# endiqq/Multi-Feature-ViT

Hardware: AMD Instinct MI355X
Metric: images/sec (two-stream 224^2 vit_small MF-CA train step) (higher is better)
Workload: dtype bf16x3 (split bf16 hi+lo operands, 3 MFMAs per product, f32 accumulate)

## Files before the change

### include/mfvit.h

```cpp
#ifndef MFVIT_H
#define MFVIT_H
#include <stddef.h>
#include <stdint.h>

#ifdef __cplusplus
extern "C" {
#endif

typedef void* mfvit_stream_t;

#define MFVIT_OK 0
#define MFVIT_EINVAL (-22)
#define MFVIT_ENOSYS (-38)
#define MFVIT_ELAUNCH (-5)

#define MFVIT_F32 0
#define MFVIT_BF16 1
#define MFVIT_BF16X3 2
#define MFVIT_F16 3
#define MFVIT_X3F16 4

int mfvit_abi_version(void);
const char* mfvit_build_info(void);

typedef struct mfvit_vit_cfg {
    int dtype;
    int batch;
    int img_h, img_w;
    int dim;
    int depth;
    int heads;
    int mlp_dim;
    int save_for_backward;
    int stop_grad_conv1;
    float ln_eps;
    int token_input;
    int tokens;
    int use_pos;
    int act;
    float p_embd, p_attn, p_resid;
    uint32_t seed_lo, seed_hi;
    int stream_share;
} mfvit_vit_cfg;

size_t mfvit_vit_param_count(const mfvit_vit_cfg* cfg);
int mfvit_vit_param_layout(const mfvit_vit_cfg* cfg, int64_t out[9]);

size_t mfvit_vit_shadow_bytes(const mfvit_vit_cfg* cfg);
int mfvit_vit_prepare_shadow(const mfvit_vit_cfg* cfg, const float* params, void* shadow, mfvit_stream_t stream);

size_t mfvit_vit_workspace_bytes(const mfvit_vit_cfg* cfg);

int mfvit_vit_forward(const mfvit_vit_cfg* cfg, const float* params, const void* shadow, const float* img, void* workspace,
                      float* features, mfvit_stream_t stream);

int mfvit_vit_backward(const mfvit_vit_cfg* cfg, const float* params, const void* shadow, void* workspace, const float* dfeatures,
                       float* dparams, int stage_hi, int stage_lo, mfvit_stream_t stream);

typedef struct mfvit_vit_drop {
    float drop;
    float attn_drop;
    const float* drop_path;
    uint64_t seed;
} mfvit_vit_drop;
size_t mfvit_vit_workspace_bytes_drop(const mfvit_vit_cfg* cfg, const mfvit_vit_drop* drop);
int mfvit_vit_forward_drop(const mfvit_vit_cfg* cfg, const mfvit_vit_drop* drop, const float* params, const void* shadow, const float* img,
                           void* workspace, float* features, mfvit_stream_t stream);
int mfvit_vit_backward_drop(const mfvit_vit_cfg* cfg, const mfvit_vit_drop* drop, const float* params, const void* shadow, void* workspace,
                            const float* dfeatures, float* dparams, int stage_hi, int stage_lo, mfvit_stream_t stream);

size_t mfvit_vit_workspace_bytes_ex(const mfvit_vit_cfg* cfg, const mfvit_vit_drop* drop, int want_dimg);
int mfvit_vit_backward_ex(const mfvit_vit_cfg* cfg, const mfvit_vit_drop* drop, const float* params, const void* shadow, void* workspace,
                          const float* dfeatures, float* dparams, float* dimg, int stage_hi, int stage_lo, mfvit_stream_t stream);

typedef struct mfvit_vit_attn_req {
    uint64_t blocks;
    int fuse;
    int cls_only;
    float* maps;
    float* rollout;
    void* scratch;
} mfvit_vit_attn_req;
size_t mfvit_vit_attn_scratch_bytes(const mfvit_vit_cfg* cfg, const mfvit_vit_attn_req* req);
int mfvit_vit_forward_attn(const mfvit_vit_cfg* cfg, const mfvit_vit_attn_req* req, const float* params, const void* shadow,
                           const float* img, void* workspace, float* features, mfvit_stream_t stream);

typedef struct mfvit_vit_rel_req {
    uint64_t blocks;
    float* maps;
    float* relevance;
    void* scratch;
} mfvit_vit_rel_req;
size_t mfvit_vit_rel_scratch_bytes(const mfvit_vit_cfg* cfg, const mfvit_vit_rel_req* req);
int mfvit_vit_backward_rel(const mfvit_vit_cfg* cfg, const mfvit_vit_rel_req* req, const float* params, const void* shadow, void* workspace,
                           const float* dfeatures, mfvit_stream_t stream);

int mfvit_gpt_forward(const mfvit_vit_cfg* cfg, const float* params, const void* shadow, const float* tokens, void* workspace, float* out,
                      mfvit_stream_t stream);
int mfvit_gpt_backward(const mfvit_vit_cfg* cfg, const float* params, const void* shadow, void* workspace, const float* dout, float* dparams,
                       float* dtokens, mfvit_stream_t stream);

int mfvit_linear_fwd(int dtype, int epilogue, const void* x, int64_t ldx, const void* w, int64_t ldw, const float* bias, void* y,
                     int64_t ldy, void* y2, int64_t ldy2, int M, int N, int K, mfvit_stream_t stream);
int mfvit_linear_dgrad_act(int dtype, const void* dy, int64_t lddy, const void* wt, int64_t ldwt, const void* act_grad, int64_t ldg,
                           void* dx, int64_t lddx, int M, int N, int K, mfvit_stream_t stream);
int mfvit_linear_wgrad(int dtype, const void* dy, int64_t lddy, const void* x, int64_t ldx, float* dw, int64_t lddw, int M, int N, int K,
                       mfvit_stream_t stream);
#define MFVIT_WGRAD_SCRATCH_FLOATS (384 * 128 * 128)
int mfvit_linear_wgrad_ws(int dtype, const void* dy, int64_t lddy, const void* x, int64_t ldx, float* dw, int64_t lddw, int M, int N,
                          int K, float* scratch, mfvit_stream_t stream);
int mfvit_linear_wgrad_pair(int dtype, const void* dy_a, int64_t lddy_a, const void* x_a, int64_t ldx_a, float* dw_a, int64_t lddw_a, float* dbias_a,
                            int Na, const void* dy_b, int64_t lddy_b, const void* x_b, int64_t ldx_b, float* dw_b, int64_t lddw_b, int Nb, int M, int K,
                            mfvit_stream_t stream);
int mfvit_linear_res_ln_fwd(int dtype, const void* a, int64_t lda, const void* w, int64_t ldw, const float* bias, const float* res,
                            int64_t ldres, float* x_out, void* y, int y_f32, const float* gamma, const float* beta, float eps,
                            float* mean, float* rstd, int M, int K, mfvit_stream_t stream);
int mfvit_linear_dgrad_ln_bwd(int dtype, const void* dy, int64_t lddy, const void* wt, int64_t ldwt, const float* x, const float* mean,
                              const float* rstd, const float* gamma, const float* dres, float* dx, void* dx_t, float* dgamma,
                              float* dbeta, float* dcol, int M, int K, mfvit_stream_t stream);
#define MFVIT_ROWP_SCRATCH_FLOATS (264 * 7 * 12 * 512)
int mfvit_linear_res_ln_fwd_ws(int dtype, const void* a, int64_t lda, const void* w, int64_t ldw, const float* bias, const float* res,
                               int64_t ldres, float* x_out, void* y, int y_f32, const float* gamma, const float* beta, float eps,
                               float* mean, float* rstd, int M, int K, float* scratch, mfvit_stream_t stream);
int mfvit_linear_dgrad_ln_bwd_ws(int dtype, const void* dy, int64_t lddy, const void* wt, int64_t ldwt, const float* x, const float* mean,
                                 const float* rstd, const float* gamma, const float* dres, float* dx, void* dx_t, float* dgamma,
                                 float* dbeta, float* dcol, int M, int K, float* scratch, mfvit_stream_t stream);
int mfvit_attention_qkv_dtype(int dtype, int T, int head_dim);
int mfvit_attention_fwd(int dtype, const void* qkv, void* out, float* lse, int B, int T, int H, int head_dim, mfvit_stream_t stream);
int mfvit_attention_bwd(int dtype, const void* qkv, const void* out, const void* dout, const float* lse, void* dqkv, float* dbias_qkv,
                        int B, int T, int H, int head_dim, mfvit_stream_t stream);
int mfvit_attention_drop_fwd(int dtype, const void* qkv, void* out, float* lse, int B, int T, int H, int head_dim, float p, uint64_t seed,
                             uint32_t site, mfvit_stream_t stream);
int mfvit_attention_drop_bwd(int dtype, const void* qkv, const void* out, const void* dout, const float* lse, void* dqkv, int B, int T, int H,
                             int head_dim, float p, uint64_t seed, uint32_t site, mfvit_stream_t stream);
int mfvit_dropout_mask(float p, uint64_t seed, uint32_t site, int64_t n, uint8_t* keep, mfvit_stream_t stream);
int mfvit_layernorm_fwd(int dtype, const float* x, void* y, int y_f32, const float* gamma, const float* beta, float eps, float* mean,
                        float* rstd, int rows, int N, mfvit_stream_t stream);
int mfvit_layernorm_bwd(int dtype, const float* dy, const float* x, const float* mean, const float* rstd, const float* gamma,
                        const float* dres, float* dx, void* dx_t, float* dgamma, float* dbeta, float* dcol, int rows, int N,
                        mfvit_stream_t stream);
int mfvit_cast_transpose(int dtype, const float* src, void* dst, void* dst_t, int R, int C, mfvit_stream_t stream);
int mfvit_head_fwd(const float* x, int64_t ldx, const float* w, const float* b, float* y, int64_t ldy, int M, int N, int K, int accumulate,
                   mfvit_stream_t stream);
int mfvit_head_bwd(const float* dy, int64_t lddy, const float* x, int64_t ldx, const float* w, float* dx, int64_t lddx, int dx_accumulate,
                   float* dw, float* db, int M, int N, int K, mfvit_stream_t stream);
int mfvit_cross_entropy(const float* logits, const int64_t* target, float* loss_mean, float* dlogits, int64_t* preds, int B, int C,
                        mfvit_stream_t stream);
int mfvit_cross_entropy_soft(const float* logits, const int64_t* target, const int32_t* partner, const float* lam, float smoothing,
                             float* loss_mean, float* dlogits, int64_t* preds, int B, int C, mfvit_stream_t stream);

int mfvit_batch_mix(const float* a, const float* b, float* out_a, float* out_b, const int32_t* desc, const float* lam, int n, int C, int H,
                    int W, mfvit_stream_t stream);

int mfvit_input_transform(const uint8_t* src, const int64_t* desc, const int32_t* tables, int n, int S, int crop, const float* mean3,
                          const float* std3, float* out, mfvit_stream_t stream);
int mfvit_input_transform_rect(const uint8_t* src, const int64_t* desc, const int32_t* tables, int n, int S, int out_h, int out_w,
                               const float* mean3, const float* std3, float* out, mfvit_stream_t stream);

size_t mfvit_input_photometric_workspace_bytes(int n, int S);
int mfvit_input_photometric(const uint8_t* src, const int64_t* desc, const int32_t* tables, const int32_t* photo, int n, int S, int max_radius,
                            void* workspace, const float* mean3, const float* std3, float* out, mfvit_stream_t stream);

int mfvit_eval_counts(const float* scores, int64_t ld, const int64_t* labels, int n, int C, uint64_t* confusion, int64_t* preds,
                      uint64_t* u2, uint64_t* npos, mfvit_stream_t stream);

typedef struct mfvit_fusion_cfg {
    int batch;
    int tokens;
    int dim;
    int heads;
    int num_classes;
    float eps_pre;
    float eps_post;
} mfvit_fusion_cfg;

size_t mfvit_fusion_param_count(const mfvit_fusion_cfg* cfg);
size_t mfvit_fusion_workspace_bytes(const mfvit_fusion_cfg* cfg);
int mfvit_fusion_forward(const mfvit_fusion_cfg* cfg, const float* params, const float* f_cxr, const float* f_enh, const float* hw_cxr,
                         const float* hb_cxr, const float* hw_enh, const float* hb_enh, void* workspace, float* fused, float* x_cxr,
                         float* x_enh, mfvit_stream_t stream);
int mfvit_fusion_backward(const mfvit_fusion_cfg* cfg, const float* params, const float* f_cxr, const float* f_enh, const float* hw_cxr,
                          const float* hw_enh, void* workspace, const float* dfused, const float* dx_cxr, const float* dx_enh,
                          float* dparams, float* df_cxr, float* df_enh, float* dhw_cxr, float* dhb_cxr, float* dhw_enh, float* dhb_enh,
                          mfvit_stream_t stream);

size_t mfvit_fusion_ex_param_count(const mfvit_fusion_cfg* cfg, int cross_attn_depth, int pool_mean);
size_t mfvit_fusion_ex_workspace_bytes(const mfvit_fusion_cfg* cfg, int cross_attn_depth, int pool_mean);
int mfvit_fusion_ex_forward(const mfvit_fusion_cfg* cfg, int cross_attn_depth, int pool_mean, const float* params, const float* f_cxr,
                            const float* f_enh, const float* hw_cxr, const float* hb_cxr, const float* hw_enh, const float* hb_enh,
                            void* workspace, float* fused, float* x_cxr, float* x_enh, mfvit_stream_t stream);
int mfvit_fusion_ex_backward(const mfvit_fusion_cfg* cfg, int cross_attn_depth, int pool_mean, const float* params, const float* f_cxr,
                             const float* f_enh, const float* hw_cxr, const float* hw_enh, void* workspace, const float* dfused,
                             const float* dx_cxr, const float* dx_enh, float* dparams, float* df_cxr, float* df_enh, float* dhw_cxr,
                             float* dhb_cxr, float* dhw_enh, float* dhb_enh, mfvit_stream_t stream);

int mfvit_prenorm_xattn_forward(const mfvit_fusion_cfg* cfg, const float* params, const float* x_own, const float* x_oth,
                                void* workspace, float* out, mfvit_stream_t stream);
int mfvit_prenorm_xattn_backward(const mfvit_fusion_cfg* cfg, const float* params, const float* x_own, const float* x_oth,
                                 void* workspace, const float* dout, float* dparams, float* dx_own, float* dx_oth,
                                 mfvit_stream_t stream);

int mfvit_xattn_forward(const mfvit_fusion_cfg* cfg, const float* params, const float* x, void* workspace, float* out,
                        mfvit_stream_t stream);
int mfvit_xattn_backward(const mfvit_fusion_cfg* cfg, const float* params, const float* x, void* workspace, const float* dout,
                         float* dparams, float* dx, mfvit_stream_t stream);

int mfvit_prof_enable(int class_mask);
int mfvit_set_wgrad_stream(int enabled);
int mfvit_set_stream_share(int n);
int mfvit_prof_collect(double* out, int ncls);
int mfvit_prof_collect_tags(double* out, int ntags);
const char* mfvit_prof_class_name(int cls);

int mfvit_bn_stats(int dtype, const void* x, int n, int C, float* mean, float* m2, mfvit_stream_t stream);
int mfvit_bn_combine(const float* means, const float* m2s, const float* counts, int W, int C, float eps, float momentum, float* mean,
                     float* invstd, float* running_mean, float* running_var, mfvit_stream_t stream);
int mfvit_bn_apply(int dtype, const void* x, const float* mean, const float* invstd, const float* gamma, const float* beta, int relu,
                   void* y, int n, int C, mfvit_stream_t stream);
int mfvit_bn_bwd_sums(int dtype, const void* dy, const void* x, const void* y, const float* mean, const float* invstd, int relu, int n,
                      int C, float* s1, float* s2, mfvit_stream_t stream);
int mfvit_bn_bwd_apply(int dtype, const void* dy, const void* x, const void* y, const float* mean, const float* invstd, const float* gamma,
                       int relu, const float* S1, const float* S2, float inv_count, void* dx, int n, int C, mfvit_stream_t stream);
int mfvit_l2norm_fwd(const float* x, float* y, float* inv_norm, int n, int C, float eps, mfvit_stream_t stream);
int mfvit_l2norm_bwd(const float* dy, const float* y, const float* inv_norm, float* dx, int n, int C, mfvit_stream_t stream);
int mfvit_rowdot(const float* a, const float* b, float* out, int64_t ldo, float scale, int n, int C, mfvit_stream_t stream);
int mfvit_cross_entropy_rows(const float* logits, int64_t ld, const int64_t* target, float* loss_mean, float* lse, float* dlogits,
// ... 21 lines not shown
```

### multi-feature-vit_amd/csrc/elementwise.hip

```cpp
#include "kernels.h"

namespace mfvit {

template <typename T>
__global__ void im2col16_kernel(const float* __restrict__ img, T* __restrict__ P, int B, int Hh, int Ww) {
    const int gh = Hh / 16, gw = Ww / 16;
    const long total = (long)B * gh * gw * 3 * 16 * 2;
    for (long q = blockIdx.x * (long)blockDim.x + threadIdx.x; q < total; q += (long)gridDim.x * blockDim.x) {
        const int half = q & 1;
        long r = q >> 1;
        const int py = r % 16; r /= 16;
        const int c = r % 3; r /= 3;
        const int pw = r % gw; r /= gw;
        const int ph = r % gh; r /= gh;
        const int b = (int)r;
        const float* s = img + (((long)b * 3 + c) * Hh + ph * 16 + py) * Ww + pw * 16 + half * 8;
        const float4 v0 = *(const float4*)s, v1 = *(const float4*)(s + 4);
        const int k = c * 256 + py * 16 + half * 8;
        T* d = P + ((long)(b * gh + ph) * gw + pw) * 768 * elems_per<T>::value + (is_split<T>::value ? split_col(k) : k);
        if constexpr (sizeof(T) == 2) {
            typedef typename Vec4<T>::elem E;
            const float f[8] = {v0.x, v0.y, v0.z, v0.w, v1.x, v1.y, v1.z, v1.w};
            typename Vec8<T>::type o, l;
#pragma unroll
// ... 395 lines not shown
#pragma unroll
    for (int k = 0; k < 4; ++k) {
        const int q = threadIdx.x + 256 * k, r = q >> 4, c = (q & 15) * 4;
        float4 v = make_float4(0.f, 0.f, 0.f, 0.f);
        if (r0 + r < R && c0 + c < C) {
            v = *(const float4*)(src + (long)(r0 + r) * C + c0 + c);
            if (dst) store_elem4<T>(dst + (long)(r0 + r) * C * elems_per<T>::value, c0 + c, v.x, v.y, v.z, v.w);
        }
        tile[r][c] = v.x;
        tile[r][c + 1] = v.y;
        tile[r][c + 2] = v.z;
        tile[r][c + 3] = v.w;
    }
    __syncthreads();
    if (dstT) {
#pragma unroll
        for (int k = 0; k < 4; ++k) {
            const int q = threadIdx.x + 256 * k, c = q >> 4, r = (q & 15) * 4;
            if (r0 + r < R && c0 + c < C)
                store_elem4<T>(dstT + (long)(c0 + c) * R * elems_per<T>::value, r0 + r, tile[r][c], tile[r + 1][c], tile[r + 2][c], tile[r + 3][c]);
        }
    }
}
int cast_transpose_batched(int dtype, const float* src, void* dst, void* dstT, int R, int C, int nb, long s_src, long s_dst, long s_dstT,
                           hipStream_t st) {
    const dim3 grid((C + 63) / 64, (R + 63) / 64, nb);
    if (R % 4 == 0 && C % 4 == 0 && s_src % 4 == 0 && s_dst % 16 == 0 && s_dstT % 16 == 0 &&
        (((uintptr_t)src | (uintptr_t)dst | (uintptr_t)dstT) & 15) == 0 && !(dtype == MFVIT_BF16X3 && ((dst && C % 32) || (dstT && R % 32)))) {
        switch (dtype) {
            case MFVIT_BF16: MFVIT_LAUNCH(cast_transpose4_kernel<bf16>, grid, dim3(256), 0, st, src, (bf16*)dst, (bf16*)dstT, R, C, s_src, s_dst, s_dstT); break;
            case MFVIT_BF16X3: MFVIT_LAUNCH(cast_transpose4_kernel<sbf16>, grid, dim3(256), 0, st, src, (sbf16*)dst, (sbf16*)dstT, R, C, s_src, s_dst, s_dstT); break;
            case MFVIT_F16: MFVIT_LAUNCH(cast_transpose4_kernel<f16>, grid, dim3(256), 0, st, src, (f16*)dst, (f16*)dstT, R, C, s_src, s_dst, s_dstT); break;
            case MFVIT_F32: MFVIT_LAUNCH(cast_transpose4_kernel<float>, grid, dim3(256), 0, st, src, (float*)dst, (float*)dstT, R, C, s_src, s_dst, s_dstT); break;
            default: return MFVIT_EINVAL;
        }
        MFVIT_CHECK_LAUNCH();
        return MFVIT_OK;
    }
    if (dtype == MFVIT_BF16)
        MFVIT_LAUNCH(cast_transpose_kernel<bf16>, grid, dim3(256), 0, st, src, (bf16*)dst, (bf16*)dstT, R, C, s_src, s_dst, s_dstT);
    else if (dtype == MFVIT_BF16X3) {
        if ((dst && C % 32) || (dstT && R % 32)) return MFVIT_EINVAL;
        MFVIT_LAUNCH(cast_transpose_kernel<sbf16>, grid, dim3(256), 0, st, src, (sbf16*)dst, (sbf16*)dstT, R, C, s_src, s_dst, s_dstT);
    } else if (dtype == MFVIT_F16)
        MFVIT_LAUNCH(cast_transpose_kernel<f16>, grid, dim3(256), 0, st, src, (f16*)dst, (f16*)dstT, R, C, s_src, s_dst, s_dstT);
    else if (dtype == MFVIT_F32)
        MFVIT_LAUNCH(cast_transpose_kernel<float>, grid, dim3(256), 0, st, src, (float*)dst, (float*)dstT, R, C, s_src, s_dst, s_dstT);
    else
        return MFVIT_EINVAL;
    MFVIT_CHECK_LAUNCH();
    return MFVIT_OK;
}
int cast_transpose(int dtype, const float* src, void* dst, void* dstT, int R, int C, hipStream_t st) {
    return cast_transpose_batched(dtype, src, dst, dstT, R, C, 1, 0, 0, 0, st);
}

__global__ __launch_bounds__(256) void linear_small_fwd_kernel(const float* __restrict__ x, long ldx, const float* __restrict__ W,
                                                               const float* __restrict__ b, float* __restrict__ y, long ldy, int M, int N,
                                                               int K, int accumulate) {
    const int o = blockIdx.x * 4 + (threadIdx.x >> 6), lane = threadIdx.x & 63;
    if (o >= M * N) return;
    const int m = o / N, n = o % N;
    float s = 0.f;
    for (int k = lane; k < K; k += 64) s = fmaf(x[(long)m * ldx + k], W[(long)n * K + k], s);
    s = wave_sum(s);
    if (lane == 0) {
        s += b ? b[n] : 0.f;
        if (accumulate) y[(long)m * ldy + n] += s; else y[(long)m * ldy + n] = s;
    }
}
__global__ __launch_bounds__(256) void linear_small_bwd_kernel(const float* __restrict__ dy, long lddy, const float* __restrict__ x, long ldx,
                                                               const float* __restrict__ W, float* __restrict__ dx, long lddx,
                                                               int dx_accumulate, float* __restrict__ dW, float* __restrict__ db, int M,
                                                               int N, int K) {
    const long id = blockIdx.x * (long)blockDim.x + threadIdx.x;
    if (dx && id < (long)M * K) {
        const int m = id / K, k = id % K;
        float s = 0.f;
        for (int n = 0; n < N; ++n) s = fmaf(dy[(long)m * lddy + n], W[(long)n * K + k], s);
        if (dx_accumulate) dx[(long)m * lddx + k] += s; else dx[(long)m * lddx + k] = s;
    }
    if (dW && id < (long)N * K) {
        const int n = id / K, k = id % K;
        float s = 0.f;
        for (int m = 0; m < M; ++m) s = fmaf(dy[(long)m * lddy + n], x[(long)m * ldx + k], s);
        dW[(long)n * K + k] += s;
    }
    if (db && id < N) {
        float s = 0.f;
        for (int m = 0; m < M; ++m) s += dy[(long)m * lddy + id];
        db[id] += s;
    }
}
int linear_small_fwd(const float* x, long ldx, const float* W, const float* b, float* y, long ldy, int M, int N, int K, int accumulate,
                     hipStream_t st) {
    MFVIT_LAUNCH(linear_small_fwd_kernel, dim3((M * N + 3) / 4), dim3(256), 0, st, x, ldx, W, b, y, ldy, M, N, K, accumulate);
    MFVIT_CHECK_LAUNCH();
    return MFVIT_OK;
}
int linear_small_bwd(const float* dy, long lddy, const float* x, long ldx, const float* W, float* dx, long lddx, int dx_accumulate, float* dW,
                     float* db, int M, int N, int K, hipStream_t st) {
    long work = (long)M * K;
    if ((long)N * K > work) work = (long)N * K;
    MFVIT_LAUNCH(linear_small_bwd_kernel, dim3((unsigned)((work + 255) / 256)), dim3(256), 0, st, dy, lddy, x, ldx, W, dx, lddx,
                       dx_accumulate, dW, db, M, N, K);
    MFVIT_CHECK_LAUNCH();
    return MFVIT_OK;
}

__global__ __launch_bounds__(1024) void ce_small_kernel(const float* __restrict__ logits, const long* __restrict__ target, float* __restrict__ loss_mean,
                                                        float* __restrict__ dlogits, long* __restrict__ preds, int B, int C) {
    __shared__ float red[16];
    float li = 0.f;
    for (int b = threadIdx.x; b < B; b += 1024) {
        const float* z = logits + (long)b * C;
        float m = z[0];
        int am = 0;
        for (int c = 1; c < C; ++c) if (z[c] > m) { m = z[c]; am = c; }
        float s = 0.f;
        for (int c = 0; c < C; ++c) s += __expf(z[c] - m);
        const float lse = m + __logf(s);
        const int t = (int)target[b];
        li += (lse - z[t]) / (float)B;
        if (dlogits)
            for (int c = 0; c < C; ++c) dlogits[(long)b * C + c] = (__expf(z[c] - lse) - (c == t ? 1.f : 0.f)) / (float)B;
        if (preds) preds[b] = am;
    }
    li = wave_sum(li);
    if ((threadIdx.x & 63) == 0) red[threadIdx.x >> 6] = li;
    __syncthreads();
    if (threadIdx.x == 0) {
        float t = 0.f;
#pragma unroll
        for (int i = 0; i < 16; ++i) t += red[i];
        *loss_mean = t;
    }
}
int ce_small(const float* logits, const long* target, float* loss_mean, float* dlogits, long* preds, int B, int C, hipStream_t st) {
    if (C > 64 || C < 1) return MFVIT_EINVAL;
    MFVIT_LAUNCH(ce_small_kernel, dim3(1), dim3(1024), 0, st, logits, target, loss_mean, dlogits, preds, B, C);
    MFVIT_CHECK_LAUNCH();
    return MFVIT_OK;
}

__global__ void add_rows_kernel(float* __restrict__ dst, long ldd, const float* __restrict__ src, long lds_, int rows, int N) {
    const long id = blockIdx.x * (long)blockDim.x + threadIdx.x;
    if (id < (long)rows * N) dst[(id / N) * ldd + id % N] += src[(id / N) * lds_ + id % N];
}
int add_rows(float* dst, long ldd, const float* src, long lds_, int rows, int N, hipStream_t st) {
    MFVIT_LAUNCH(add_rows_kernel, dim3((unsigned)(((long)rows * N + 255) / 256)), dim3(256), 0, st, dst, ldd, src, lds_, rows, N);
    MFVIT_CHECK_LAUNCH();
    return MFVIT_OK;
}
__global__ void axpy_kernel(float* __restrict__ y, const float* __restrict__ x, float a, long n) {
    const long i = blockIdx.x * (long)blockDim.x + threadIdx.x;
    if (i < n) y[i] = fmaf(a, x[i], y[i]);
}
int axpy(float* y, const float* x, float a, long n, hipStream_t st) {
    MFVIT_LAUNCH(axpy_kernel, dim3((unsigned)((n + 255) / 256)), dim3(256), 0, st, y, x, a, n);
    MFVIT_CHECK_LAUNCH();
    return MFVIT_OK;
}
__global__ __launch_bounds__(1024) void colsum_rows_kernel(const float* __restrict__ x, long ld, float* __restrict__ out, int rows,
                                                           int row_stride, int row_off, int N) {
    const int n = blockIdx.x * 64 + (threadIdx.x & 63), sub = threadIdx.x >> 6;
    __shared__ float sm[16][64];
    float s = 0.f;
    if (n < N) {
#pragma unroll 4
        for (int r = sub; r < rows; r += 16) s += x[((long)r * row_stride + row_off) * ld + n];
    }
    sm[sub][threadIdx.x & 63] = s;
    __syncthreads();
    if (sub == 0 && n < N) {
        s = 0.f;
#pragma unroll
        for (int i = 0; i < 16; ++i) s += sm[i][threadIdx.x];
        out[n] += s;
    }
}
int colsum_rows(const float* x, long ld, float* out, int rows, int row_stride, int row_off, int N, hipStream_t st) {
    MFVIT_LAUNCH(colsum_rows_kernel, dim3((N + 63) / 64), dim3(1024), 0, st, x, ld, out, rows, row_stride, row_off, N);
    MFVIT_CHECK_LAUNCH();
    return MFVIT_OK;
}

__global__ __launch_bounds__(256) void batch_sum_kernel(const float* __restrict__ x, float* __restrict__ out, int B, long n) {
    const long i = blockIdx.x * 256L + threadIdx.x;
    if (i >= n) return;
    float s = 0.f;
    for (int b = 0; b < B; ++b) s += x[(long)b * n + i];
    out[i] += s;
}
int batch_sum(const float* x, float* out, int B, long n, hipStream_t st) {
    MFVIT_LAUNCH(batch_sum_kernel, dim3((unsigned)((n + 255) / 256)), dim3(256), 0, st, x, out, B, n);
    MFVIT_CHECK_LAUNCH();
    return MFVIT_OK;
}

__global__ __launch_bounds__(256) void dropout_mask_kernel(DropP drop, long n, unsigned char* __restrict__ out) {
    const long i = (long)blockIdx.x * 256 + threadIdx.x;
    if (i < n) out[i] = drop_mul(drop, (unsigned)i) != 0.f;
}
int dropout_mask(DropP drop, long n, unsigned char* out, hipStream_t st) {
    if (n <= 0 || n >= (1L << 32)) return MFVIT_EINVAL;
    MFVIT_LAUNCH(dropout_mask_kernel, dim3((unsigned)((n + 255) / 256)), dim3(256), 0, st, drop, n, out);
    MFVIT_CHECK_LAUNCH();
    return MFVIT_OK;
}

}
```

### multi-feature-vit_amd/csrc/gemm.hip

```cpp
#include "kernels.h"
#include "prof.h"

#include <stdlib.h>

#include <type_traits>

namespace mfvit {




template <typename T, int EPI, int DEEP = 0>
__global__ __launch_bounds__(256, 2) void gemm_nt_tile_kernel(GemmP p) {
    constexpr int BM = 128, BN = 128, BKB = 128, WM = 2, WN = 2, NTHR = WM * WN * 64;
    typedef NtLoop<T, BM, BN, BKB, WM, WN> Loop;
    extern __shared__ __attribute__((aligned(16))) char lds[];
    apply_batch<T>(p, sizeof(T));
    const int ntn = p.N / BN;
    const int ntm = (p.M + BM - 1) / BM;
    const int bid = xcd_remap(blockIdx.x, ntn * ntm);
    const int m0 = (bid / ntn) * BM, n0 = (bid % ntn) * BN;
    f32x16 acc[Loop::TM][Loop::TN];
    if constexpr (DEEP == 12) {
        NtLoopDeep<T, BM, BN, BKB, WM, WN, 2, true>::run(p, m0, n0, lds, acc);
// ... 739 lines not shown
    typedef STile<T, BN, KR> TA;
    typedef STile<T, BK2, KR> TB;
    constexpr int STAGE = TA::BYTES + TB::BYTES;
    extern __shared__ __attribute__((aligned(16))) char lds[];
    apply_batch<T>(p, 4);
    const int tid = threadIdx.x, lane = tid & 63, wave = tid >> 6;
    const int wm = wave >> 1, wn = wave & 1;
    constexpr bool SPLIT = is_split<T>::value;
    constexpr int EP = elems_per<T>::value;
    const int ntk = p.K * EP / BK2;
    int tile = blockIdx.x, split = blockIdx.y;
    if (gridDim.y == 1 && p.splits > 1) {
        const int tiles = ntk * (p.N * EP / BN);
        const int lin = xcd_remap(blockIdx.x, gridDim.x);
        split = lin / tiles;
        tile = lin % tiles;
    }
    const int n0 = (tile / ntk) * BN, k0 = (tile % ntk) * BK2;
    int chunk = (p.M + p.splits - 1) / p.splits;
    chunk = (chunk + KR - 1) / KR * KR;
    const int mbeg = split * chunk;
    const int mend = min(p.M, mbeg + chunk);
    if (mbeg >= mend) return;
    const T* A = (const T*)p.A;
    const T* X = (const T*)p.W;
    SStage<T, BN, KR, NT> sa;
    SStage<T, BK2, KR, NT> sb;
    f32x16 acc[2][2];
#pragma unroll
    for (int i = 0; i < 2; ++i)
#pragma unroll
        for (int j = 0; j < 2; ++j)
#pragma unroll
            for (int r = 0; r < 16; ++r) acc[i][j][r] = 0.f;
    const bool do_cs = p.cs0 != nullptr && k0 == 0 && wn == 0;
    f32x16 bacc[2];
    typename MmaTraits<T>::frag_t ones;
    if constexpr (sizeof(T) == 2) {
        typedef typename Vec4<T>::elem E16;
#pragma unroll
        for (int j = 0; j < 8; ++j) ones[j] = (E16)1.0f;
    } else {
        ones = 1.0f;
    }
#pragma unroll
    for (int i = 0; i < 2; ++i)
#pragma unroll
        for (int r = 0; r < 16; ++r) bacc[i][r] = 0.f;
    const int nst = (mend - mbeg + KR - 1) / KR;
    const int nfull = (mend - mbeg) / KR;
    auto load_stage = [&](int stg) {
        if (stg < nfull) {
            sa.template load<REMAP, false>(A, p.lda, mbeg + stg * KR, mend, n0, tid, p.orow_in, p.orow_out, p.orow_off);
            sb.template load<false, false>(X, p.ldw, mbeg + stg * KR, mend, k0, tid);
        } else {
            sa.template load<REMAP, true>(A, p.lda, mbeg + stg * KR, mend, n0, tid, p.orow_in, p.orow_out, p.orow_off);
            sb.template load<false, true>(X, p.ldw, mbeg + stg * KR, mend, k0, tid);
        }
    };
    auto main_loop = [&](auto cs_tag) {
        constexpr bool CS = decltype(cs_tag)::value;
        load_stage(0);
        sa.store(lds, tid);
        sb.store(lds + TA::BYTES, tid);
        __syncthreads();
        int cur = 0;
        for (int st = 0; st < nst; ++st) {
            const char* ta = lds + cur * STAGE;
            const char* tb = ta + TA::BYTES;
            if (st + 1 < nst) load_stage(st + 1);
            typename MmaTraits<T>::frag_t a[2][2], b[2][2];
#pragma unroll
            for (int i = 0; i < 2; ++i) a[0][i] = TA::frag(ta, (wm * 2 + i) * 32, 0, lane);
#pragma unroll
            for (int j = 0; j < 2; ++j) b[0][j] = TB::frag(tb, (wn * 2 + j) * 32, 0, lane);
#pragma unroll
            for (int s = 0; s < TA::KSTEPS; ++s) {
                if (s + 1 < TA::KSTEPS) {
#pragma unroll
                    for (int i = 0; i < 2; ++i) a[(s + 1) & 1][i] = TA::frag(ta, (wm * 2 + i) * 32, s + 1, lane);
#pragma unroll
                    for (int j = 0; j < 2; ++j) b[(s + 1) & 1][j] = TB::frag(tb, (wn * 2 + j) * 32, s + 1, lane);
                }
                __builtin_amdgcn_sched_barrier(0);
#pragma unroll
                for (int i = 0; i < 2; ++i)
#pragma unroll
                    for (int j = 0; j < 2; ++j)
                        if (!(SPLIT && i == 1 && j == 1)) acc[i][j] = MmaTraits<T>::mma(a[s & 1][i], b[s & 1][j], acc[i][j]);
                if constexpr (CS) {
#pragma unroll
                    for (int i = 0; i < 2; ++i) bacc[i] = MmaTraits<T>::mma(a[s & 1][i], ones, bacc[i]);
                }
                __builtin_amdgcn_sched_barrier(0);
            }
            if (st + 1 < nst) {
                char* na = lds + (cur ^ 1) * STAGE;
                sa.store(na, tid);
                sb.store(na + TA::BYTES, tid);
            }
            __syncthreads();
            cur ^= 1;
        }
    };
    if (do_cs) main_loop(std::true_type{});
    else main_loop(std::false_type{});
    if constexpr (SPLIT) {
#pragma unroll
        for (int r = 0; r < 16; ++r) {
            acc[0][0][r] += acc[0][1][r] + acc[1][0][r];
            bacc[0][r] += bacc[1][r];
        }
    }
    constexpr int NI = SPLIT ? 1 : 2;
    const int nw = SPLIT ? n0 / 2 + wm * 32 : n0 + wm * 64, kw = SPLIT ? k0 / 2 + wn * 32 : k0 + wn * 64;
    if (p.cpart) {
        float* part = p.cpart + (long)split * p.N * p.K;
#pragma unroll
        for (int i = 0; i < NI; ++i)
#pragma unroll
            for (int j = 0; j < NI; ++j)
#pragma unroll
                for (int r = 0; r < 16; ++r) {
                    const int n = nw + i * 32 + acc_row(r, lane);
                    const int k = kw + j * 32 + (lane & 31);
                    part[(long)n * p.K + k] = acc[i][j][r];
                }
    } else {
        float* out = (float*)p.out0;
#pragma unroll
        for (int i = 0; i < NI; ++i)
#pragma unroll
            for (int j = 0; j < NI; ++j)
#pragma unroll
                for (int r = 0; r < 16; ++r) {
                    const int n = nw + i * 32 + acc_row(r, lane);
                    const int k = kw + j * 32 + (lane & 31);
                    atomicAdd(out + (long)n * p.ldo0 + k, acc[i][j][r]);
                }
    }
    if (do_cs && (lane & 31) == 0) {
#pragma unroll
        for (int i = 0; i < NI; ++i)
#pragma unroll
            for (int r = 0; r < 16; ++r) {
                const int n = nw + i * 32 + acc_row(r, lane);
                if (p.kpart) p.kpart[(long)split * p.N + n] = bacc[i][r];
                else atomicAdd(p.cs0 + n, bacc[i][r]);
            }
    }
}

__global__ __launch_bounds__(256) void tn_reduce_kernel(const float* __restrict__ part, int splits, long stride, int N, int K, float* __restrict__ out,
                                                        long ldo) {
    const long q = (long)blockIdx.x * 256 + threadIdx.x;
    const long total4 = (long)N * K / 4;
    if (q >= total4) return;
    const long e = q * 4;
    float4 s = *(const float4*)(part + e);
    for (int t = 1; t < splits; ++t) {
        const float4 v = *(const float4*)(part + (long)t * stride + e);
        s.x += v.x, s.y += v.y, s.z += v.z, s.w += v.w;
    }
    const int n = (int)(e / K), k = (int)(e % K);
    float4* o = (float4*)(out + (long)n * ldo + k);
    float4 c = *o;
    c.x += s.x, c.y += s.y, c.z += s.z, c.w += s.w;
    *o = c;
}
__global__ __launch_bounds__(256) void tn_reduce_batch_kernel(TnPartBatch b) {
    const long q = (long)blockIdx.x * 256 + threadIdx.x;
    if (q >= b.total4) return;
    int lo = 0, hi = b.n - 1;
    while (lo < hi) {
        const int mid = (lo + hi + 1) >> 1;
        if (b.job[mid].first4 <= q) lo = mid; else hi = mid - 1;
    }
    const TnPartJob& j = b.job[lo];
    const long e = (q - j.first4) * 4;
    float4 s = *(const float4*)(j.part + e);
    for (int t = 1; t < j.splits; ++t) {
        const float4 v = *(const float4*)(j.part + (long)t * j.stride + e);
        s.x += v.x, s.y += v.y, s.z += v.z, s.w += v.w;
    }
    const int n = (int)(e / j.K), k = (int)(e % j.K);
    float4* o = (float4*)(j.out + (long)n * j.ldo + k);
    float4 c = *o;
    c.x += s.x, c.y += s.y, c.z += s.z, c.w += s.w;
    *o = c;
}

template <typename T, int EPI> static int launch_tile(const GemmP& pin, hipStream_t st) {
    typedef NtLoop<T, 128, 128, 128, 2, 2> Loop;
    GemmP p = pin;
    constexpr int EP = elems_per<T>::value;
    if (p.N % 128 || p.K * EP % Loop::BK || p.M <= 0) return MFVIT_EINVAL;
    if (p.omax && (EPI != EPI_NONE || p.omax_rows < 64 || p.M % p.omax_rows || (p.omax_hd != 32 && p.omax_hd != 64) || p.nb > 1)) return MFVIT_EINVAL;
    const int nwg = (p.N / 128) * ((p.M + 127) / 128);
    constexpr int epi_bytes = 128 * ((EPI == EPI_COL2IM16 ? 128 * 4 : 128 * (int)sizeof(T) * EP) + 16);
    constexpr int lds_bytes = Loop::LDS_BYTES > epi_bytes ? Loop::LDS_BYTES : epi_bytes;
    static PerDeviceOnce attr_set;
    if (attr_set.first()) {
        (void)hipFuncSetAttribute((const void*)gemm_nt_tile_kernel<T, EPI>, hipFuncAttributeMaxDynamicSharedMemorySize, lds_bytes);
        if constexpr (sizeof(T) == 2 && !is_split<T>::value)
            (void)hipFuncSetAttribute((const void*)gemm_nt_tile_kernel<T, EPI, 2>, hipFuncAttributeMaxDynamicSharedMemorySize, lds_bytes);
    }
    ProfScope ps(PROF_GEMM_TILE, 2.0 * p.M * p.N * p.K * (p.nb > 1 ? p.nb : 1), 0, st);
    if constexpr (sizeof(T) == 2) {
        const bool fits = (unsigned long long)(p.M - 1) * p.lda * 2 + 256 < (1ull << 32) && (unsigned long long)(p.N - 1) * p.ldw * 2 + 256 < (1ull << 32);
        const bool deep_ok = p.K * EP / Loop::BK >= 2 && (p.K * EP / Loop::BK) % 2 == 0 && fits;
        if constexpr (is_split<T>::value) {
            if (deep_ok) {
                static PerDeviceOnce a12;
                if (a12.first())
                    (void)hipFuncSetAttribute((const void*)gemm_nt_tile_kernel<T, EPI, 12>, hipFuncAttributeMaxDynamicSharedMemorySize, lds_bytes);
                MFVIT_LAUNCH((gemm_nt_tile_kernel<T, EPI, 12>), dim3(nwg, 1, p.nb > 1 ? p.nb : 1), dim3(256), lds_bytes, st, p);
                MFVIT_CHECK_LAUNCH();
                return MFVIT_OK;
            }
        } else if (deep_ok) {
            MFVIT_LAUNCH((gemm_nt_tile_kernel<T, EPI, 2>), dim3(nwg, 1, p.nb > 1 ? p.nb : 1), dim3(256), lds_bytes, st, p);
            MFVIT_CHECK_LAUNCH();
            return MFVIT_OK;
        }
    }
    MFVIT_LAUNCH((gemm_nt_tile_kernel<T, EPI>), dim3(nwg, 1, p.nb > 1 ? p.nb : 1), dim3(256), lds_bytes, st, p);
    MFVIT_CHECK_LAUNCH();
    return MFVIT_OK;
}
static int row_grid(const GemmP& p, int BM) {
    const int rpw = p.rows_per_wg > 0 ? p.rows_per_wg : BM;
    return (p.M + rpw - 1) / rpw;
}
template <typename T, int REPI, int WM, int BKB, int BM> static int launch_row_v(const GemmP& pin, hipStream_t st) {
    GemmP p = pin;
    p.rows_per_wg = 0;
    typedef NtLoop<T, BM, ROW_BN, BKB, WM, 4> Loop;
    if (p.N != ROW_BN || p.K * elems_per<T>::value % Loop::BK || p.M <= 0) return MFVIT_EINVAL;
    constexpr int need = BM * ROW_RS * 4 + BM * 4;
    constexpr int need2 = WM * 3 * ROW_BN * 4;
    constexpr int bytes0 = Loop::LDS_BYTES > need ? Loop::LDS_BYTES : need;
    constexpr int bytes1 = bytes0 > need2 ? bytes0 : need2;
    constexpr bool lean = WM == 1 && sizeof(T) == 2 && BM == 64;
    constexpr int bytes = lean && ROW_LEAN_LDS > bytes1 ? ROW_LEAN_LDS : bytes1;
    static PerDeviceOnce attr_set;
    if (attr_set.first()) {
        (void)hipFuncSetAttribute((const void*)gemm_nt_row_kernel<T, REPI, WM, BKB, BM>, hipFuncAttributeMaxDynamicSharedMemorySize, bytes);
    }
    ProfScope ps(REPI == REPI_RES_LN ? PROF_GEMM_ROW_FWD : PROF_GEMM_ROW_BWD, 2.0 * p.M * p.N * p.K, 0, st);
    MFVIT_LAUNCH((gemm_nt_row_kernel<T, REPI, WM, BKB, BM>), dim3(row_grid(p, BM)), dim3(WM * 256), bytes, st, p);
    MFVIT_CHECK_LAUNCH();
    return MFVIT_OK;
}
template <typename T, int REPI> static int launch_row(const GemmP& p, hipStream_t st) {
    if constexpr (sizeof(T) == 2) {
        if (p.M > 256 * 64 || p.K * elems_per<T>::value % (128 / (int)sizeof(T))) return launch_row_v<T, REPI, 1, 64, 64>(p, st);
    } else {
        if (p.K % (128 / (int)sizeof(T))) return launch_row_v<T, REPI, 1, 64, 64>(p, st);
    }
    if constexpr (REPI == REPI_RES_LN) {
        if (p.K >= 768 && p.M >= 128 * 128) return launch_row_v<T, REPI, 2, 128, 128>(p, st);
    }
    return launch_row_v<T, REPI, 2, 128, 64>(p, st);
}
template <typename T> static int launch_tn(GemmP p, hipStream_t st) {
    constexpr int EP = elems_per<T>::value;
    if (p.N * EP % 128 || p.K * EP % 128 || p.M <= 0) return MFVIT_EINVAL;
    constexpr int KR = 128 / (int)sizeof(T);
    const int tiles = (p.N * EP / 128) * (p.K * EP / 128);
    if (p.splits <= 0) {
        constexpr int target = 384;
        int s = (tiles >= 16 ? target : (target * 2) / 3) / tiles;
        const int maxs = (p.M + 4 * KR - 1) / (4 * KR);
        p.splits = s < 1 ? 1 : (s > maxs ? maxs : s);
    }
    {
        int chunk = (p.M + p.splits - 1) / p.splits;
        chunk = (chunk + KR - 1) / KR * KR;
        p.splits = (p.M + chunk - 1) / chunk;
    }
    const bool xcd1d = p.splits > 1 && p.nb <= 1;
    constexpr int bytes = 2 * (STile<T, 128, KR>::BYTES * 2);
    static PerDeviceOnce attr_set;
    if (attr_set.first()) {
        (void)hipFuncSetAttribute((const void*)gemm_tn_kernel<T, false>, hipFuncAttributeMaxDynamicSharedMemorySize, bytes);
        (void)hipFuncSetAttribute((const void*)gemm_tn_kernel<T, true>, hipFuncAttributeMaxDynamicSharedMemorySize, bytes);
    }
    if (p.nb > 1 || p.splits < 2 || p.ldo0 % 4 || (long)tiles * p.splits > 384) p.cpart = nullptr;
    p.kpart = p.cpart && p.cs0 && (long)tiles * p.splits + 2 <= 384 && p.N % 4 == 0 && (size_t)p.cs0 % 16 == 0 ? p.cpart + (long)p.splits * p.N * p.K : nullptr;
    ProfScope ps(PROF_GEMM_TN, 2.0 * p.M * p.N * p.K * (p.nb > 1 ? p.nb : 1), 0, st);
    const dim3 grid = xcd1d ? dim3(tiles * p.splits, 1, 1) : dim3(tiles, p.splits, p.nb > 1 ? p.nb : 1);
    if (p.orow_in)
        MFVIT_LAUNCH((gemm_tn_kernel<T, true>), grid, dim3(256), bytes, st, p);
    else
        MFVIT_LAUNCH((gemm_tn_kernel<T, false>), grid, dim3(256), bytes, st, p);
    MFVIT_CHECK_LAUNCH();
    if (p.cpart) {
        const int rc = tn_partial_reduce(p.cpart, p.splits, (long)p.N * p.K, p.N, p.K, (float*)p.out0, p.ldo0, st);
        if (rc != MFVIT_OK || !p.kpart) return rc;
        return tn_partial_reduce(p.kpart, p.splits, p.N, 1, p.N, p.cs0, p.N, st);
    }
    return MFVIT_OK;
}

static thread_local TnPartBatch* g_tnpart_batch = nullptr;
TnPartBatch* tnpart_batch_begin(TnPartBatch* b) {
    TnPartBatch* prev = g_tnpart_batch;
    if (b) { b->n = 0; b->total4 = 0; }
    g_tnpart_batch = b;
    return prev;
}
int tnpart_batch_flush(hipStream_t st) {
    TnPartBatch* b = g_tnpart_batch;
    if (!b || b->n == 0) return MFVIT_OK;
    MFVIT_LAUNCH(tn_reduce_batch_kernel, dim3((unsigned)((b->total4 + 255) / 256)), dim3(256), 0, st, *b);
    b->n = 0;
    b->total4 = 0;
    MFVIT_CHECK_LAUNCH();
    return MFVIT_OK;
}
int tn_partial_reduce(const float* part, int splits, long stride, int N, int K, float* out, long ldo, hipStream_t st) {
    if (TnPartBatch* b = g_tnpart_batch) {
        if (b->n == TnPartBatch::MAXJ) {
            const int rc = tnpart_batch_flush(st);
            if (rc != MFVIT_OK) return rc;
        }
        TnPartJob& j = b->job[b->n++];
        j.part = part; j.out = out; j.stride = stride; j.ldo = ldo; j.splits = splits; j.N = N; j.K = K; j.first4 = b->total4;
        b->total4 += (long)N * K / 4;
        return MFVIT_OK;
    }
    const long total4 = (long)N * K / 4;
    MFVIT_LAUNCH(tn_reduce_kernel, dim3((unsigned)((total4 + 255) / 256)), dim3(256), 0, st, part, splits, stride, N, K, out, ldo);
    MFVIT_CHECK_LAUNCH();
    return MFVIT_OK;
}

constexpr int CPR_SUB = 16;
__device__ __forceinline__ float colpart_rows(const float* __restrict__ part, int G, long pitch, int c, int sub, float (*sm)[64]) {
    float s = 0.f;
#pragma unroll 4
    for (int g2 = sub; g2 < G; g2 += CPR_SUB) s += part[(long)g2 * pitch + c];
    sm[sub][threadIdx.x & 63] = s;
    __syncthreads();
    s = 0.f;
    if (sub == 0) {
#pragma unroll
        for (int i = 0; i < CPR_SUB; ++i) s += sm[i][threadIdx.x];
    }
    return s;
}
__global__ __launch_bounds__(64 * CPR_SUB) void colpart_reduce_kernel(const float* __restrict__ part, int G, int ncols, int nq, float* d0, float* d1,
                                                                     float* d2) {
    const int c = blockIdx.x * 64 + (threadIdx.x & 63), sub = threadIdx.x >> 6;
    __shared__ float sm[CPR_SUB][64];
    const bool ok = c < nq * ncols;
    float s = colpart_rows(part, ok ? G : 0, (long)nq * ncols, c, sub, sm);
    if (sub == 0 && ok) {
        float* d = c / ncols == 0 ? d0 : (c / ncols == 1 ? d1 : d2);
        if (d) atomicAdd(d + c % ncols, s);
    }
}
#define MFVIT_TRY_RC(expr) do { int rc__ = (expr); if (rc__ != MFVIT_OK) return rc__; } while (0)
__global__ __launch_bounds__(64 * CPR_SUB) void colpart_reduce_batch_kernel(ColpartBatch b) {
    const ColpartJob& j = b.job[blockIdx.z];
    const int c = blockIdx.x * 64 + (threadIdx.x & 63), sub = threadIdx.x >> 6;
    __shared__ float sm[CPR_SUB][64];
    const bool ok = c < j.nq * j.ncols;
    float s = colpart_rows(j.part, ok ? j.G : 0, (long)j.nq * j.ncols, c, sub, sm);
    if (sub == 0 && ok) {
        float* d = j.d[c / j.ncols];
        if (d) atomicAdd(d + c % j.ncols, s);
    }
}
static thread_local ColpartBatch* g_colpart_batch = nullptr;
ColpartBatch* colpart_batch_begin(ColpartBatch* b) {
    ColpartBatch* prev = g_colpart_batch;
    if (b) b->n = 0;
    g_colpart_batch = b;
    return prev;
}
int colpart_batch_flush(hipStream_t st) {
    ColpartBatch* b = g_colpart_batch;
    if (!b || b->n == 0) return MFVIT_OK;
    int cmax = 0;
    for (int i = 0; i < b->n; ++i) cmax = b->job[i].nq * b->job[i].ncols > cmax ? b->job[i].nq * b->job[i].ncols : cmax;
    MFVIT_LAUNCH(colpart_reduce_batch_kernel, dim3((cmax + 63) / 64, 1, b->n), dim3(64 * CPR_SUB), 0, st, *b);
    b->n = 0;
    MFVIT_CHECK_LAUNCH();
    return MFVIT_OK;
}
int colpart_reduce(const float* part, int G, int ncols, int nq, float* d0, float* d1, float* d2, hipStream_t st) {
    if (ColpartBatch* b = g_colpart_batch) {
        if (b->n == ColpartBatch::MAXJ) MFVIT_TRY_RC(colpart_batch_flush(st));
        ColpartJob& j = b->job[b->n++];
        j.part = part; j.G = G; j.ncols = ncols; j.nq = nq; j.d[0] = d0; j.d[1] = d1; j.d[2] = d2;
        return MFVIT_OK;
    }
    MFVIT_LAUNCH(colpart_reduce_kernel, dim3((nq * ncols + 63) / 64), dim3(64 * CPR_SUB), 0, st, part, G, ncols, nq, d0, d1, d2);
    MFVIT_CHECK_LAUNCH();
    return MFVIT_OK;
}

#define MFVIT_BY_DTYPE(dtype, CALL)                       \
    switch (dtype) {                                      \
        case MFVIT_F32: { typedef float TT; return CALL; }    \
        case MFVIT_BF16: { typedef bf16 TT; return CALL; }    \
        case MFVIT_BF16X3: { typedef sbf16 TT; return CALL; } \
        case MFVIT_F16: { typedef f16 TT; return CALL; }      \
        default: return MFVIT_EINVAL;                     \
    }
template <int EPI> static int tile_by_dtype(int dtype, const GemmP& p, hipStream_t st) { MFVIT_BY_DTYPE(dtype, (launch_tile<TT, EPI>(p, st))) }
template <int REPI> static int row_by_dtype(int dtype, const GemmP& p, hipStream_t st) { MFVIT_BY_DTYPE(dtype, (launch_row<TT, REPI>(p, st))) }
static int tn_by_dtype(int dtype, const GemmP& p, hipStream_t st) { MFVIT_BY_DTYPE(dtype, (launch_tn<TT>(p, st))) }

int gemm_nt_tile(int dtype, int epi, const GemmP& p, hipStream_t st) {
    if (gemm_nt_pp_supported(dtype, epi, p)) return gemm_nt_pp(dtype, epi, p, st);
    if (epi == EPI_GELU_BWD && p.cpart && p.cs0) {
        const int rc = tile_by_dtype<EPI_GELU_BWD>(dtype, p, st);
        if (rc != MFVIT_OK) return rc;
        return colpart_reduce(p.cpart, (p.M + 127) / 128, p.N, 1, p.cs0, nullptr, nullptr, st);
    }
    if (gemm_nt_small_supported(dtype, epi, p)) return gemm_nt_small(epi, p, st);
    switch (epi) {
        case EPI_BIAS: return tile_by_dtype<EPI_BIAS>(dtype, p, st);
        case EPI_BIAS_GELU: return tile_by_dtype<EPI_BIAS_GELU>(dtype, p, st);
        case EPI_GELU_BWD: return tile_by_dtype<EPI_GELU_BWD>(dtype, p, st);
        case EPI_NONE: return tile_by_dtype<EPI_NONE>(dtype, p, st);
        case EPI_BIAS_RELU: return tile_by_dtype<EPI_BIAS_RELU>(dtype, p, st);
        case EPI_BIAS_X3F16: return dtype == MFVIT_BF16X3 ? launch_tile<sbf16, EPI_BIAS_X3F16>(p, st) : MFVIT_EINVAL;
        case EPI_COL2IM16:
            if (!p.out0 || p.nb > 1 || p.N != 768 || p.ldo0 <= 0 || p.ldo0 % 16 || p.orow_in <= 0 || p.orow_out <= p.orow_in || p.orow_in % (p.ldo0 / 16))
                return MFVIT_EINVAL;
            return tile_by_dtype<EPI_COL2IM16>(dtype, p, st);
        case EPI_BIAS_GELU_DROP:
            switch (dtype) {
                case MFVIT_BF16: return launch_tile<bf16, EPI_BIAS_GELU_DROP>(p, st);
                case MFVIT_BF16X3: return launch_tile<sbf16, EPI_BIAS_GELU_DROP>(p, st);
                case MFVIT_F16: return launch_tile<f16, EPI_BIAS_GELU_DROP>(p, st);
            }
            return MFVIT_EINVAL;
    }
    return MFVIT_EINVAL;
}
int gemm_nt_row(int dtype, int repi, const GemmP& p, hipStream_t st) {
    if (gemm_nt_rowp_supported(dtype, repi, p)) return gemm_nt_rowp(dtype, repi, p, st);
    if (repi == REPI_RES_LN) return row_by_dtype<REPI_RES_LN>(dtype, p, st);
    if (repi == REPI_LNBWD_RES) {
        const int rc = row_by_dtype<REPI_LNBWD_RES>(dtype, p, st);
        if (rc != MFVIT_OK || !p.cpart) return rc;
        GemmP q = p;
        q.rows_per_wg = 0;
        return colpart_reduce(p.cpart, row_grid(q, 64), ROW_BN, 3, p.cs0, p.cs1, p.cs2, st);
    }
    return MFVIT_EINVAL;
}
int gemm_tn(int dtype, const GemmP& p, hipStream_t st) {
    if (gemm_tn_glds_supported(dtype, p)) return gemm_tn_glds(dtype, p, st);
    {
        GemmP q = p;
        q.cpart = nullptr;
        if (gemm_tn_small_supported(dtype, q)) return gemm_tn_small(q, st);
    }
    return tn_by_dtype(dtype, p, st);
}

}
```

### multi-feature-vit_amd/csrc/gemm_small.hip

```cpp
#include "gemm.cuh"
#include "kernels.h"
#include "prof.h"

namespace mfvit {

namespace {

constexpr int SM_MAX_ROWS = 512;

__device__ __forceinline__ f32x16 mma_f32(float a, float b, f32x16 c) { return __builtin_amdgcn_mfma_f32_32x32x2f32(a, b, c, 0, 0, 0); }

__device__ __forceinline__ void reduce_waves(f32x16& acc, float* red, int wave, int lane) {
    if (wave) {
#pragma unroll
        for (int r = 0; r < 16; ++r) red[((wave - 1) * 16 + r) * 64 + lane] = acc[r];
    }
    __syncthreads();
    if (!wave) {
#pragma unroll
        for (int w = 0; w < 3; ++w)
#pragma unroll
            for (int r = 0; r < 16; ++r) acc[r] += red[(w * 16 + r) * 64 + lane];
    }
}

template <int STEPS>
__global__ __launch_bounds__(256) void gemm_nt_small_kernel(GemmP p) {
    __shared__ float red[3 * 16 * 64];
    apply_batch<float>(p, 4);
    const int lane = threadIdx.x & 63, wave = threadIdx.x >> 6;
    const int r = lane & 31, hh = lane >> 5;
    const int n0 = blockIdx.x * 32, m0 = blockIdx.y * 32;
    const int kc = p.K >> 2;
    const bool aok = m0 + r < p.M, wok = n0 + r < p.N;
    const float* ap = (const float*)p.A + (long)(aok ? m0 + r : 0) * p.lda + wave * kc + hh * 4;
    const float* wp = (const float*)p.W + (long)(wok ? n0 + r : 0) * p.ldw + wave * kc + hh * 4;
    f32x16 acc;
#pragma unroll
    for (int i = 0; i < 16; ++i) acc[i] = 0.f;
    if constexpr (STEPS > 0) {
        float4 a[STEPS], w[STEPS];
#pragma unroll
        for (int s = 0; s < STEPS; ++s) {
            a[s] = *(const float4*)(ap + 8 * s);
            w[s] = *(const float4*)(wp + 8 * s);
        }
#pragma unroll
        for (int s = 0; s < STEPS; ++s) {
            acc = mma_f32(aok ? a[s].x : 0.f, wok ? w[s].x : 0.f, acc);
            acc = mma_f32(aok ? a[s].y : 0.f, wok ? w[s].y : 0.f, acc);
            acc = mma_f32(aok ? a[s].z : 0.f, wok ? w[s].z : 0.f, acc);
            acc = mma_f32(aok ? a[s].w : 0.f, wok ? w[s].w : 0.f, acc);
        }
    } else {
        auto mma4 = [&](const float4& a, const float4& w) __attribute__((always_inline)) {
            acc = mma_f32(aok ? a.x : 0.f, wok ? w.x : 0.f, acc);
            acc = mma_f32(aok ? a.y : 0.f, wok ? w.y : 0.f, acc);
            acc = mma_f32(aok ? a.z : 0.f, wok ? w.z : 0.f, acc);
            acc = mma_f32(aok ? a.w : 0.f, wok ? w.w : 0.f, acc);
        };
        const int nch = kc >> 5;
        float4 a[4], w[4], an[4], wn[4];
        if (nch > 0) {
#pragma unroll
            for (int s = 0; s < 4; ++s) { a[s] = *(const float4*)(ap + 8 * s); w[s] = *(const float4*)(wp + 8 * s); }
        }
        for (int c = 0; c < nch; ++c) {
            const int kn = (c + 1 < nch ? c + 1 : c) * 32;
#pragma unroll
            for (int s = 0; s < 4; ++s) { an[s] = *(const float4*)(ap + kn + 8 * s); wn[s] = *(const float4*)(wp + kn + 8 * s); }
#pragma unroll
            for (int s = 0; s < 4; ++s) mma4(a[s], w[s]);
#pragma unroll
            for (int s = 0; s < 4; ++s) { a[s] = an[s]; w[s] = wn[s]; }
        }
        for (int k = nch * 32; k < kc; k += 8) mma4(*(const float4*)(ap + k), *(const float4*)(wp + k));
    }
    reduce_waves(acc, red, wave, lane);
    if (wave) return;
    const int n = n0 + r;
    if (n >= p.N) return;
    const float b = p.bias ? p.bias[n] : 0.f;
    float* out = (float*)p.out0;
#pragma unroll
    for (int i = 0; i < 16; ++i) {
        const int m = m0 + acc_row(i, lane);
        if (m < p.M) out[(long)m * p.ldo0 + n] = acc[i] + b;
    }
}

__global__ __launch_bounds__(256) void gemm_tn_small_kernel(GemmP p) {
    __shared__ float red[3 * 16 * 64];
    apply_batch<float>(p, 4);
    const int lane = threadIdx.x & 63, wave = threadIdx.x >> 6;
    const int r = lane & 31, hh = lane >> 5;
    const int k0 = blockIdx.x * 32, n0 = blockIdx.y * 32;
    const int mc = ((p.M + 3) / 4 + 1) & ~1;
    const int mb = wave * mc, me = min(p.M, mb + mc);
    const bool aok = n0 + r < p.N, wok = k0 + r < p.K;
    const float* ap = (const float*)p.A + (aok ? n0 + r : 0);
    const float* wp = (const float*)p.W + (wok ? k0 + r : 0);
    f32x16 acc;
#pragma unroll
    for (int i = 0; i < 16; ++i) acc[i] = 0.f;
    for (int m = mb + hh; m < mb + mc + hh; m += 8) {
        float a[4], w[4];
#pragma unroll
        for (int j = 0; j < 4; ++j) {
            const int mj = m + 2 * j;
            const bool in = mj < me;
            const long mm = in ? mj : 0;
            a[j] = ap[mm * p.lda];
            if (!in || !aok) a[j] = 0.f;
            w[j] = wok ? wp[mm * p.ldw] : 0.f;
        }
#pragma unroll
        for (int j = 0; j < 4; ++j) acc = mma_f32(a[j], w[j], acc);
    }
    reduce_waves(acc, red, wave, lane);
    if (wave) return;
    const int k = k0 + r;
    if (k >= p.K) return;
    float* out = (float*)p.out0;
#pragma unroll
    for (int i = 0; i < 16; ++i) {
        const int n = n0 + acc_row(i, lane);
        if (n < p.N) atomicAdd(out + (long)n * p.ldo0 + k, acc[i]);
    }
}

bool plain(const GemmP& p) {
    return !p.out1 && !p.aux && !p.res && !p.res_t && !p.orow_in && !p.gamma && !p.cs0 && !p.cs1 && !p.cs2 && !p.cpart && !p.omax && p.out0 && p.A && p.W;
}
bool small_switch() { return true; }

}

bool gemm_nt_small_supported(int dtype, int epi, const GemmP& p) {
    if (dtype != MFVIT_F32 || (epi != EPI_NONE && epi != EPI_BIAS) || !plain(p) || !small_switch()) return false;
    if (p.M <= 0 || p.M > SM_MAX_ROWS || p.K % 32 || p.lda % 4 || p.ldw % 4) return false;
    if ((((uintptr_t)p.A | (uintptr_t)p.W) & 15) || ((p.sAo | p.sAi | p.sWo | p.sWi) & 3)) return false;
    return epi == EPI_NONE || p.bias != nullptr;
}
int gemm_nt_small(int epi, GemmP p, hipStream_t st) {
    if (epi == EPI_NONE) p.bias = nullptr;
    const int nb = p.nb > 1 ? p.nb : 1;
    ProfScope ps(PROF_OTHER, 2.0 * p.M * p.N * p.K * nb, 0, st);
    const dim3 grid((p.N + 31) / 32, (p.M + 31) / 32, nb);
    if (p.K == 384)
        MFVIT_LAUNCH(gemm_nt_small_kernel<12>, grid, dim3(256), 0, st, p);
    else if (p.K == 128)
        MFVIT_LAUNCH(gemm_nt_small_kernel<4>, grid, dim3(256), 0, st, p);
    else
        MFVIT_LAUNCH(gemm_nt_small_kernel<0>, grid, dim3(256), 0, st, p);
    MFVIT_CHECK_LAUNCH();
    return MFVIT_OK;
}

bool gemm_tn_small_supported(int dtype, const GemmP& p) {
    return dtype == MFVIT_F32 && plain(p) && !p.bias && small_switch() && p.M > 0 && p.M <= SM_MAX_ROWS;
}
int gemm_tn_small(GemmP p, hipStream_t st) {
    const int nb = p.nb > 1 ? p.nb : 1;
    ProfScope ps(PROF_OTHER, 2.0 * p.M * p.N * p.K * nb, 0, st);
    MFVIT_LAUNCH(gemm_tn_small_kernel, dim3((p.K + 31) / 32, (p.N + 31) / 32, nb), dim3(256), 0, st, p);
    MFVIT_CHECK_LAUNCH();
    return MFVIT_OK;
}

}
```

### multi-feature-vit_amd/csrc/gemm_tn2.hip

```cpp
#include <stdlib.h>

#include <type_traits>
#include "gemm.cuh"
#include "kernels.h"
#include "prof.h"

namespace mfvit {

namespace {

constexpr int T2_NS = 3;
constexpr int T2_NSP = 4;
constexpr int T2_TILE = 16 * 1024;
constexpr int T2_STAGE = 2 * T2_TILE;

template <typename T> struct T2Geo {
    static constexpr bool SPLIT = is_split<T>::value;
    static constexpr int TW = SPLIT ? 256 : 128;
    static constexpr int KR = SPLIT ? 32 : 64;
    static constexpr int ROWB = TW * 2;
    static constexpr int CPR = ROWB / 16;
    static constexpr int RPI = 64 / CPR;
    static constexpr int NF = TW / 2 / 32;
    static constexpr int BL = 128;
// ... 208 lines not shown
            for (int j = 0; j < NF; ++j) b[0][j] = t2_frag<T>(tb, (wn * NF + j) * 32, sb0, lane);
#pragma unroll
            for (int s = 0; s < KS; ++s) {
                if (s + 1 < KS) {
#pragma unroll
                    for (int i = 0; i < NF; ++i) a[(s + 1) & 1][i] = t2_frag<T>(ta, (wm * NF + i) * 32, sb0 + s + 1, lane);
#pragma unroll
                    for (int j = 0; j < NF; ++j) b[(s + 1) & 1][j] = t2_frag<T>(tb, (wn * NF + j) * 32, sb0 + s + 1, lane);
                }
                constexpr int MPK = SPLIT ? 3 * NL * NL : NL * NL;
                constexpr int NM = KS * MPK, ND = 2 * NI;
#pragma unroll
                for (int t = 0; t < MPK; ++t) {
                    const int term = t / (NL * NL), i = (t % (NL * NL)) / NL, j = t % NL;
                    if constexpr (SPLIT)
                        acc[i][j] = MmaTraits<T>::mma(a[s & 1][2 * i + (term == 0 ? 1 : 0)], b[s & 1][2 * j + (term == 1 ? 1 : 0)], acc[i][j]);
                    else
                        acc[i][j] = MmaTraits<T>::mma(a[s & 1][i], b[s & 1][j], acc[i][j]);
                    if constexpr (IL) {
                        const int m = s * MPK + t;
                        if ((m + 1) * ND / NM != m * ND / NM) dma_one(st + 2, nslot, m * ND / NM);
                        __builtin_amdgcn_sched_barrier(0);
                    }
                }
                if constexpr (WITH_CS) {
                    {
                        if constexpr (SPLIT) {
                            const frag_t ch = wn ? a[s & 1][2] : a[s & 1][0], cl = wn ? a[s & 1][3] : a[s & 1][1];
                            bacc[0] = MmaTraits<T>::mma(ch, ones, bacc[0]);
                            bacc[0] = MmaTraits<T>::mma(cl, ones, bacc[0]);
                        } else {
                            const frag_t ch = wn ? a[s & 1][1] : a[s & 1][0];
                            bacc[0] = MmaTraits<T>::mma(ch, ones, bacc[0]);
                        }
                    }
                }
            }
            asm volatile("s_waitcnt lgkmcnt(0)" ::: "memory");
            slot = slot == T2_NS - 1 ? 0 : slot + 1;
        }
        if constexpr (IL) t2_wait_vm<0>();
    };
    if constexpr (SPLIT && W8 && IL) {
        if (do_cs) main_loop_pipe(std::true_type{});
        else main_loop_pipe(std::false_type{});
    } else {
        if (do_cs) main_loop(std::true_type{});
        else main_loop(std::false_type{});
    }
    const int nw = n0 / EP + wm * 64, kw = k0 / EP + wn * 64;
    float* out = (float*)(second ? p.out1 : p.out0);
    const long ldo_ = second ? p.ldo1 : p.ldo0;
    if constexpr (W8) {
        __syncthreads();
        float* xch = (float*)lds + (size_t)wq * (NL * NL * 16 * 64) + lane;
        float* bxch = (float*)lds + (size_t)4 * (NL * NL * 16 * 64) + (size_t)wq * (16 * 64) + lane;
        if (CS && do_cs && kh == 1) {
#pragma unroll
            for (int r = 0; r < 16; ++r) bxch[r * 64] = bacc[0][r];
        }
        if (kh == 1) {
#pragma unroll
            for (int i = 0; i < NL; ++i)
#pragma unroll
                for (int j = 0; j < NL; ++j)
#pragma unroll
                    for (int r = 0; r < 16; ++r) xch[((i * NL + j) * 16 + r) * 64] = acc[i][j][r];
        }
        __syncthreads();
        if (kh == 0) {
#pragma unroll
            for (int i = 0; i < NL; ++i)
#pragma unroll
                for (int j = 0; j < NL; ++j)
#pragma unroll
                    for (int r = 0; r < 16; ++r) acc[i][j][r] += xch[((i * NL + j) * 16 + r) * 64];
            if (CS && do_cs) {
#pragma unroll
                for (int r = 0; r < 16; ++r) bacc[0][r] += bxch[r * 64];
            }
        }
    }
    if (!W8 || kh == 0) {
        if (p.cpart) {
            float* part = p.cpart + (long)split * (p.N + p.res_mod) * p.K + (second ? (long)p.N * p.K : 0);
#pragma unroll
            for (int i = 0; i < NL; ++i)
#pragma unroll
                for (int j = 0; j < NL; ++j)
#pragma unroll
                    for (int r = 0; r < 16; ++r) {
                        const int n = nw + i * 32 + acc_row(r, lane);
                        const int k = kw + j * 32 + (lane & 31);
                        __builtin_nontemporal_store(acc[i][j][r], part + (long)n * p.K + k);
                    }
        } else {
#pragma unroll
            for (int i = 0; i < NL; ++i)
#pragma unroll
                for (int j = 0; j < NL; ++j)
#pragma unroll
                    for (int r = 0; r < 16; ++r) {
                        const int n = nw + i * 32 + acc_row(r, lane);
                        const int k = kw + j * 32 + (lane & 31);
                        atomicAdd(out + (long)n * ldo_ + k, acc[i][j][r]);
                    }
        }
    }
    if (CS) {
        if (do_cs && (!W8 || kh == 0) && (lane & 31) == 0) {
#pragma unroll
            for (int r = 0; r < 16; ++r) {
                const int n = nw + wn * 32 + acc_row(r, lane);
                if (p.kpart) p.kpart[(long)split * p.N + n] = bacc[0][r];
                else atomicAdd(p.cs0 + n, bacc[0][r]);
            }
        }
    }
}

}

bool gemm_tn_glds_supported(int dtype, const GemmP& p) {
    static int sw_on = INT_MIN;
    if (env_switch("MFVIT_TN_GLDS", 1, sw_on) == 0 || (dtype != MFVIT_BF16 && dtype != MFVIT_BF16X3 && dtype != MFVIT_F16) || p.nb > 1) return false;
    if (p.orow_in && (dtype != MFVIT_BF16X3 || p.cs0 || p.res_mod)) return false;
    if (p.N % 128 || p.K % 128 || p.M < 2048) return false;
    if (p.lda % 8 || p.ldw % 8) return false;
    return true;
}

bool gemm_tn_pair_supported(int dtype, const GemmP& a, const GemmP& b) {
    if (!gemm_tn_glds_supported(dtype, a) || !gemm_tn_glds_supported(dtype, b)) return false;
    if (a.M != b.M || a.K != b.K || b.cs0 || b.cpart || a.splits > 0 || b.splits > 0 || a.res_mod || b.res_mod) return false;
    return true;
}

template <typename T> static int launch_t2(GemmP p, hipStream_t st) {
    typedef T2Geo<T> G;
    const int tiles = ((p.N + p.res_mod) / 128) * (p.K / 128);
    if (p.splits <= 0) {
        const int target = stream_share() >= 2 && p.M < 8192 ? 128 : 256;
        int s = target / tiles;
        const int maxs = (p.M + 4 * G::KR - 1) / (4 * G::KR);
        p.splits = s < 1 ? 1 : (s > maxs ? maxs : s);
    }
    {
        int chunk = (p.M + p.splits - 1) / p.splits;
        chunk = (chunk + G::KR - 1) / G::KR * G::KR;
        p.splits = (p.M + chunk - 1) / chunk;
    }
    if (p.splits < 2 || p.ldo0 % 4 || (p.res_mod && p.ldo1 % 4) || (long)tiles * p.splits > 384) p.cpart = nullptr;
    p.kpart = p.cpart && p.cs0 && (long)tiles * p.splits + 2 <= 384 && p.N % 4 == 0 && (size_t)p.cs0 % 16 == 0 ? p.cpart + (long)p.splits * (p.N + p.res_mod) * p.K : nullptr;
    constexpr int bytes = (is_split<T>::value ? T2_NSP : T2_NS) * T2_STAGE;
    p.rows_per_wg = 0;
    ProfScope ps(PROF_GEMM_TN, 2.0 * p.M * (p.N + p.res_mod) * p.K, 0, st);
    auto go = [&](auto cs, auto w, auto i) {
        constexpr bool CS = decltype(cs)::value, W8 = decltype(w)::value, IL = decltype(i)::value;
        static PerDeviceOnce attr;
        if (attr.first()) {
            (void)hipFuncSetAttribute((const void*)gemm_tn_glds_kernel<T, CS, W8, IL>, hipFuncAttributeMaxDynamicSharedMemorySize, bytes);
        }
        MFVIT_LAUNCH((gemm_tn_glds_kernel<T, CS, W8, IL>), dim3(tiles * p.splits), dim3(W8 ? 512 : 256), bytes, st, p);
    };
    auto go1 = [&](auto cs) { go(cs, std::true_type{}, std::true_type{}); };
    if (p.orow_in) {
        if constexpr (is_split<T>::value) {
            static PerDeviceOnce attr_rm;
            if (attr_rm.first())
                (void)hipFuncSetAttribute((const void*)gemm_tn_glds_kernel<T, false, true, true, true>, hipFuncAttributeMaxDynamicSharedMemorySize, bytes);
            MFVIT_LAUNCH((gemm_tn_glds_kernel<T, false, true, true, true>), dim3(tiles * p.splits), dim3(512), bytes, st, p);
        } else {
            return MFVIT_EINVAL;
        }
    } else if (p.cs0) go1(std::true_type{});
    else go1(std::false_type{});
    MFVIT_CHECK_LAUNCH();
    if (p.cpart) {
        const long stride = (long)(p.N + p.res_mod) * p.K;
        int rc = tn_partial_reduce(p.cpart, p.splits, stride, p.N, p.K, (float*)p.out0, p.ldo0, st);
        if (rc == MFVIT_OK && p.kpart) rc = tn_partial_reduce(p.kpart, p.splits, p.N, 1, p.N, p.cs0, p.N, st);
        if (rc != MFVIT_OK || !p.res_mod) return rc;
        return tn_partial_reduce(p.cpart + (long)p.N * p.K, p.splits, stride, p.res_mod, p.K, (float*)p.out1, p.ldo1, st);
    }
    return MFVIT_OK;
}

int gemm_tn_glds_pair(int dtype, GemmP a, const GemmP& b, hipStream_t st) {
    a.aux = b.A; a.ldaux = b.lda;
    a.res_t = b.W; a.ldres_t = b.ldw;
    a.out1 = b.out0; a.ldo1 = b.ldo0;
    a.res_mod = b.N;
    return gemm_tn_glds(dtype, a, st);
}

int gemm_tn_glds(int dtype, GemmP p, hipStream_t st) {
    if (dtype == MFVIT_BF16) return launch_t2<bf16>(p, st);
    if (dtype == MFVIT_BF16X3) return launch_t2<sbf16>(p, st);
    if (dtype == MFVIT_F16) return launch_t2<f16>(p, st);
    return MFVIT_EINVAL;
}

}
```

### multi-feature-vit_amd/csrc/kernels.h

```cpp
#pragma once
#include "gemm.cuh"

namespace mfvit {

enum { EPI_BIAS = 0, EPI_BIAS_GELU = 1, EPI_GELU_BWD = 2, EPI_NONE = 3, EPI_BIAS_RELU = 4,
       EPI_BIAS_X3F16 = 5,
       EPI_BIAS_GELU_DROP = 6,
       EPI_COL2IM16 = 7 };
enum { REPI_RES_LN = 0, REPI_LNBWD_RES = 1,
       REPI_RES_LN_DP = 2 };

int gemm_nt_tile(int dtype, int epi, const GemmP& p, hipStream_t st);
bool gemm_nt_pp_supported(int dtype, int epi, const GemmP& p);
int gemm_nt_pp(int dtype, int epi, const GemmP& p, hipStream_t st);
int gemm_nt_row(int dtype, int repi, const GemmP& p, hipStream_t st);
bool gemm_nt_rowp_supported(int dtype, int repi, const GemmP& p);
int gemm_nt_rowp(int dtype, int repi, const GemmP& p, hipStream_t st);
int input_transform(const unsigned char* src, const long long* desc, const int* tables, int n, int S, int out_h, int out_w,
                    const float* mean, const float* stdv, float* out, hipStream_t st);
int input_transform_u8(const unsigned char* src, const long long* desc, const int* tables, int n, int S, unsigned* frames,
                       hipStream_t st);
size_t input_photometric_workspace_bytes(int n, int S);
int input_photometric(const unsigned char* src, const long long* desc, const int* tables, const int* photo, int n, int S, int max_radius,
                      void* workspace, const float* mean, const float* stdv, float* out, hipStream_t st);
int eval_counts(const float* scores, long ld, const int64_t* labels, int n, int C, unsigned long long* conf, unsigned long long* u2,
                unsigned long long* npos, int64_t* preds, hipStream_t st);
int gemm_tn(int dtype, const GemmP& p, hipStream_t st);
bool gemm_nt_small_supported(int dtype, int epi, const GemmP& p);
int gemm_nt_small(int epi, GemmP p, hipStream_t st);
bool gemm_tn_small_supported(int dtype, const GemmP& p);
int gemm_tn_small(GemmP p, hipStream_t st);
bool gemm_tn_glds_supported(int dtype, const GemmP& p);
int gemm_tn_glds(int dtype, GemmP p, hipStream_t st);
int colpart_reduce(const float* part, int G, int ncols, int nq, float* d0, float* d1, float* d2, hipStream_t st);
struct ColpartJob { const float* part; float* d[3]; int G, ncols, nq; };
struct ColpartBatch { static constexpr int MAXJ = 48; int n; ColpartJob job[MAXJ]; };
ColpartBatch* colpart_batch_begin(ColpartBatch* b);
int colpart_batch_flush(hipStream_t st);
bool gemm_tn_pair_supported(int dtype, const GemmP& a, const GemmP& b);
int gemm_tn_glds_pair(int dtype, GemmP a, const GemmP& b, hipStream_t st);
int tn_partial_reduce(const float* part, int splits, long stride, int N, int K, float* out, long ldo, hipStream_t st);
struct TnPartJob { const float* part; float* out; long stride, ldo; int splits, N, K; long first4; };
struct TnPartBatch { static constexpr int MAXJ = 56; int n; long total4; TnPartJob job[MAXJ]; };
TnPartBatch* tnpart_batch_begin(TnPartBatch* b);
int tnpart_batch_flush(hipStream_t st);

int attn_fwd_exact(int dtype, const void* qkv, void* out, float* lse, int B, int Tn, int H, int HD, hipStream_t st);
int attn_bwd_exact(int dtype, const void* qkv, const void* out, const void* dout, const float* lse, void* dqkv, float* dbias, int B, int Tn,
                   int H, int HD, hipStream_t st);

int attn_qkv_dtype(int dtype, int Tn, int HD);
int attn_fwd(int dtype, const void* qkv, void* out, float* lse, int B, int Tn, int H, int HD, hipStream_t st);
int attn_bwd(int dtype, const void* qkv, const void* out, const void* dout, const float* lse, void* dqkv, float* dbias, int B, int Tn,
             int H, int HD, hipStream_t st, const unsigned* domax = nullptr);

int im2col16(int dtype, const float* img, void* P, int B, int H, int W, hipStream_t st);
int ln_rows(int dtype, int N, const float* in0, long ld0, const float* in1, long ld1, int mod1, float* xout, long ldx, void* y, long ldy,
            int y_f32, const float* gamma, const float* beta, float eps, float* mean, float* rstd, int rows, int row_stride, int row_off,
            int in0_bcast, hipStream_t st);
int ln_bwd_rows(int dtype, int N, const float* dy, long lddy, const float* x, long ldx, const float* mean, const float* rstd,
                const float* gamma, const float* dres, long ldres, float* dx, long lddx, void* dxT, long lddxT, float* dgamma, float* dbeta,
                float* dcol, float* cpart, int rows, int row_stride, int row_off, hipStream_t st, const void* dyT = nullptr, long lddyT = 0);
int add_ln_rows(int dtype, int N, const void* tin, long ldt, const float* pos, long ldp, int pmod, const float* res, long ldres, int rin, int rout,
                int roff, float* xout, long ldx, void* y, long ldy, int y_f32, const float* gamma, const float* beta, float eps, float* mean,
                float* rstd, int rows, hipStream_t st);
int cast_transpose(int dtype, const float* src, void* dst, void* dstT, int R, int C, hipStream_t st);
int cast_transpose_batched(int dtype, const float* src, void* dst, void* dstT, int R, int C, int nb, long s_src, long s_dst, long s_dstT,
                           hipStream_t st);
int linear_small_fwd(const float* x, long ldx, const float* W, const float* b, float* y, long ldy, int M, int N, int K, int accumulate,
                     hipStream_t st);
int linear_small_bwd(const float* dy, long lddy, const float* x, long ldx, const float* W, float* dx, long lddx, int dx_accumulate, float* dW,
                     float* db, int M, int N, int K, hipStream_t st);
int ce_small(const float* logits, const long* target, float* loss_mean, float* dlogits, long* preds, int B, int C, hipStream_t st);
int add_rows(float* dst, long ldd, const float* src, long lds_, int rows, int N, hipStream_t st);
int axpy(float* y, const float* x, float a, long n, hipStream_t st);
int colsum_rows(const float* x, long ld, float* out, int rows, int row_stride, int row_off, int N, hipStream_t st);
int batch_sum(const float* x, float* out, int B, long n, hipStream_t st);

int attn_fwd_tiled_drop(int dtype, const void* qkv, void* out, float* lse, int B, int Tn, int H, int HDim, DropP drop, hipStream_t st);
int attn_bwd_tiled_drop(int dtype, const void* qkv, const void* out, const void* dout, const float* lse, void* dqkv, int B, int Tn, int H, int HDim,
                        DropP drop, hipStream_t st);
bool attn_tiled_supported(int dtype, int Tn, int HDim);
int dropout_mask(DropP drop, long n, unsigned char* out, hipStream_t st);
int drop_add_ln_rows(int dtype, int N, const void* tin, long ldt, const float* a0, long lda0, const float* a1, long lda1, int mod1,
                     const float* res, long ldres, DropP drop, DropP dpath, int tpr, float* xout, long ldx, void* y, long ldy, int y_f32,
                     const float* gamma, const float* beta, float eps, float* mean, float* rstd, int rows, hipStream_t st);
int mask_scale_rows(int dtype, bool f32, const void* src, long lds_, void* dst, long ldd, DropP drop, DropP dpath, int tpr, int rows, int N,
                    hipStream_t st);
int attn_probs(int qdt, const void* qkv, const float* lse, int B, int Tn, int H, int HD, int fuse, int cls_only, float* out, float* sums,
               hipStream_t st);
int attn_rollout(const float* maps, const float* sums, int depth, int B, int Tn, float* out, hipStream_t st);
int attn_rel_map(int qdt, int ddt, const void* qkv, const float* lse, const void* dout, int B, int Tn, int H, int HD, float* map, const float* v,
                 float* part, int first, hipStream_t st);
int attn_rel_update(float* v, const float* part, int B, int Tn, int first, float* out, hipStream_t st);
}
```

### multi-feature-vit_amd/csrc/vit.hip

```cpp
#include "../../include/mfvit.h"
#include "kernels.h"
#include "prof.h"

#include <atomic>
#include <stdlib.h>
#include <string.h>

using namespace mfvit;

namespace mfvit {
static std::atomic<int> g_stream_share{1};
static thread_local int t_stream_share = 0;
int stream_share() { return t_stream_share > 0 ? t_stream_share : g_stream_share.load(std::memory_order_relaxed); }
namespace {
struct ShareScope {
    int prev;
    explicit ShareScope(const mfvit_vit_cfg* cfg) : prev(t_stream_share) { if (cfg && cfg->stream_share > 0) t_stream_share = cfg->stream_share > 8 ? 8 : cfg->stream_share; }
    ~ShareScope() { t_stream_share = prev; }
};
}
}

namespace {

// ... 418 lines not shown
        GemmP q = zero_gemm();
        q.A = ws + W.patches; q.lda = 768 * e;
        q.W = hw ? (const void*)(sh + S.pe_w) : (const void*)(params + L.pe_w); q.ldw = 768 * e;
        q.M = d.Mp; q.N = d.D; q.K = 768;
        q.bias = params + L.pe_b;
        q.out0 = ws + W.utmp; q.ldo0 = D * e;
        MFVIT_TRY(gemm_nt_tile(d.dtype, EPI_BIAS, q, st));
        MFVIT_TRY(add_ln_rows(d.dtype, d.D, ws + W.utmp, D * e, params + L.pos, D, d.T, nullptr, 0, d.np, d.T, 1, xbuf(0), D, blk(0) + W.y1, D * e, 0,
                              pblk(0) + L.ln1_w, pblk(0) + L.ln1_b, eps, stat(0), stat(0) + d.M, d.Mp, st));
    } else {
        GemmP p = zero_gemm();
        p.A = ws + W.patches; p.lda = 768 * e;
        p.W = hw ? (const void*)(sh + S.pe_w) : (const void*)(params + L.pe_w); p.ldw = 768 * e;
        p.M = d.Mp; p.N = d.D; p.K = 768;
        p.bias = params + L.pe_b;
        p.res = params + L.pos; p.ldres = D; p.res_mod = d.np; p.res_off = 1;
        p.orow_in = d.np; p.orow_out = d.T; p.orow_off = 1;
        p.out0 = xbuf(0); p.ldo0 = D;
        p.out1 = blk(0) + W.y1; p.ldo1 = D * e;
        p.gamma = pblk(0) + L.ln1_w; p.beta = pblk(0) + L.ln1_b; p.eps = eps;
        p.mean = stat(0); p.rstd = stat(0) + d.M;
        MFVIT_TRY(gemm_nt_row(d.dtype, REPI_RES_LN, p, st));
    }
    MFVIT_TRY(ln_rows(d.dtype, d.D, params + L.cls, 0, params + L.pos, D, 1, xbuf(0), D, blk(0) + W.y1, D * e, 0, pblk(0) + L.ln1_w,
                      pblk(0) + L.ln1_b, eps, stat(0), stat(0) + d.M, d.B, d.T, 0, 1, st));
    if (d.p_embd > 0.f)
        MFVIT_TRY(drop_add_ln_rows(d.dtype, d.D, nullptr, 0, xbuf(0), D, nullptr, 0, 0, nullptr, 0, make_drop(d.p_embd, d.seed, 1), off, 1, xbuf(0), D,
                                   blk(0) + W.y1, D * e, 0, pblk(0) + L.ln1_w, pblk(0) + L.ln1_b, eps, stat(0), stat(0) + d.M, d.M, st));
    }

    for (int l = 0; l < d.depth; ++l) {
        char* b = blk(l);
        const float* pb = pblk(l);
        const char* sb = sblk(l);
        const int qdt = d.p_attn > 0.f ? d.dtype : attn_qkv_dtype(d.dtype, d.T, d.HD);
        {
            GemmP p = zero_gemm();
            p.A = b + W.y1; p.lda = D * e;
            p.W = hw ? (const void*)(sb + S.qkv_w) : (const void*)(pb + L.qkv_w); p.ldw = D * e;
            p.M = d.M; p.N = 3 * d.D; p.K = d.D;
            p.bias = pb + L.qkv_b;
            p.out0 = b + W.qkv; p.ldo0 = 3 * D * e;
            ProfTag tag(PROF_TAG_MHSA_QKV);
            MFVIT_TRY(gemm_nt_tile(d.dtype, qdt == MFVIT_X3F16 ? EPI_BIAS_X3F16 : EPI_BIAS, p, st));
        }
        if (d.p_attn > 0.f) {
            if (!attn_tiled_supported(d.dtype, d.T, d.HD)) return MFVIT_ENOSYS;
            MFVIT_TRY(attn_fwd_tiled_drop(d.dtype, b + W.qkv, b + W.attn, (float*)(b + W.lse), d.B, d.T, d.H, d.HD,
                                          make_drop(d.p_attn, d.seed, site(l, 2)), st));
        } else {
            MFVIT_TRY(attn_fwd(qdt, b + W.qkv, b + W.attn, (float*)(b + W.lse), d.B, d.T, d.H, d.HD, st));
        }
        if (attn) MFVIT_TRY(attn_block_step(d, attn, l, qdt, b + W.qkv, (const float*)(b + W.lse), st));
        {
            GemmP p = zero_gemm();
            p.A = b + W.attn; p.lda = D * e;
            p.W = hw ? (const void*)(sb + S.proj_w) : (const void*)(pb + L.proj_w); p.ldw = D * e;
            p.M = d.M; p.N = d.D; p.K = d.D;
            p.bias = pb + L.proj_b;
            p.res = xbuf(l); p.ldres = D;
            p.out0 = b + W.xmid; p.ldo0 = D;
            p.out1 = b + W.y2; p.ldo1 = D * e;
            p.gamma = pb + L.ln2_w; p.beta = pb + L.ln2_b; p.eps = eps;
            p.mean = (float*)(b + W.st2); p.rstd = (float*)(b + W.st2) + d.M;
            int rc = MFVIT_OK;
            bool done;
            {
                ProfTag tag(PROF_TAG_MHSA_PROJ);
                done = rowp_dpath(p, dpath(l, 6), rc);
            }
            if (done) {
                MFVIT_TRY(rc);
            } else if (d.rdrop) {
                GemmP q = zero_gemm();
                q.A = p.A; q.lda = p.lda; q.W = p.W; q.ldw = p.ldw; q.M = p.M; q.N = p.N; q.K = p.K; q.bias = p.bias;
                q.out0 = ws + W.dtmp; q.ldo0 = D * e;
                MFVIT_TRY(gemm_nt_tile(d.dtype, EPI_BIAS, q, st));
                MFVIT_TRY(drop_add_ln_rows(d.dtype, d.D, ws + W.dtmp, D * e, nullptr, 0, nullptr, 0, 0, xbuf(l), D,
                                           make_drop(d.p_resid, d.seed, site(l, 3)), dpath(l, 6), d.T, (float*)(b + W.xmid), D, b + W.y2, D * e, 0,
                                           p.gamma, p.beta,
                                           eps, p.mean, p.rstd, d.M, st));
            } else if (d.unfused) {
                GemmP q = zero_gemm();
                q.A = p.A; q.lda = p.lda; q.W = p.W; q.ldw = p.ldw; q.M = p.M; q.N = p.N; q.K = p.K; q.bias = p.bias;
                q.out0 = ws + W.utmp; q.ldo0 = D * e;
                MFVIT_TRY(gemm_nt_tile(d.dtype, EPI_BIAS, q, st));
                MFVIT_TRY(add_ln_rows(d.dtype, d.D, ws + W.utmp, D * e, nullptr, 0, 0, xbuf(l), D, 0, 0, 0, (float*)(b + W.xmid), D, b + W.y2, D * e, 0,
                                      p.gamma, p.beta, eps, p.mean, p.rstd, d.M, st));
            } else {
                p.kpart = (float*)(ws + W.kpart);
                ProfTag tag(PROF_TAG_MHSA_PROJ);
                MFVIT_TRY(gemm_nt_row(d.dtype, REPI_RES_LN, p, st));
            }
        }
        {
            GemmP p = zero_gemm();
            p.A = b + W.y2; p.lda = D * e;
            p.W = hw ? (const void*)(sb + S.fc1_w) : (const void*)(pb + L.fc1_w); p.ldw = D * e;
            p.M = d.M; p.N = d.F; p.K = d.D;
            p.bias = pb + L.fc1_b;
            p.out0 = d.save ? b + W.hpre : nullptr; p.ldo0 = F;
            p.out1 = b + W.hact; p.ldo1 = F * e;
            p.drop = make_drop(d.p_gelu, d.seed, site(l, 5));
            MFVIT_TRY(gemm_nt_tile(d.dtype, d.act == 1 ? EPI_BIAS_RELU : (d.p_gelu > 0.f ? EPI_BIAS_GELU_DROP : EPI_BIAS_GELU), p, st));
        }
        {
            const bool last = l + 1 == d.depth;
            GemmP p = zero_gemm();
            p.A = b + W.hact; p.lda = F * e;
            p.W = hw ? (const void*)(sb + S.fc2_w) : (const void*)(pb + L.fc2_w); p.ldw = F * e;
            p.M = d.M; p.N = d.D; p.K = d.F;
            p.bias = pb + L.fc2_b;
            p.res = (const float*)(b + W.xmid); p.ldres = D;
            p.out0 = xbuf(l + 1); p.ldo0 = D;
            if (last) {
                p.out1 = features; p.ldo1 = D; p.y_f32 = 1;
                p.gamma = params + L.norm_w; p.beta = params + L.norm_b;
            } else {
                p.out1 = blk(l + 1) + W.y1; p.ldo1 = D * e;
                p.gamma = pblk(l + 1) + L.ln1_w; p.beta = pblk(l + 1) + L.ln1_b;
            }
            p.eps = eps;
            p.mean = stat(l + 1); p.rstd = stat(l + 1) + d.M;
            int rc = MFVIT_OK;
            if (rowp_dpath(p, dpath(l, 7), rc)) {
                MFVIT_TRY(rc);
            } else if (d.rdrop) {
                GemmP q = zero_gemm();
                q.A = p.A; q.lda = p.lda; q.W = p.W; q.ldw = p.ldw; q.M = p.M; q.N = p.N; q.K = p.K; q.bias = p.bias;
                q.out0 = ws + W.dtmp; q.ldo0 = D * e;
                MFVIT_TRY(gemm_nt_tile(d.dtype, EPI_BIAS, q, st));
                MFVIT_TRY(drop_add_ln_rows(d.dtype, d.D, ws + W.dtmp, D * e, nullptr, 0, nullptr, 0, 0, (const float*)(b + W.xmid), D,
                                           make_drop(d.p_resid, d.seed, site(l, 4)), dpath(l, 7), d.T, xbuf(l + 1), D, p.out1, p.ldo1, p.y_f32,
                                           p.gamma, p.beta, eps,
                                           p.mean, p.rstd, d.M, st));
            } else if (d.unfused) {
                GemmP q = zero_gemm();
                q.A = p.A; q.lda = p.lda; q.W = p.W; q.ldw = p.ldw; q.M = p.M; q.N = p.N; q.K = p.K; q.bias = p.bias;
                q.out0 = ws + W.utmp; q.ldo0 = D * e;
                MFVIT_TRY(gemm_nt_tile(d.dtype, EPI_BIAS, q, st));
                MFVIT_TRY(add_ln_rows(d.dtype, d.D, ws + W.utmp, D * e, nullptr, 0, 0, (const float*)(b + W.xmid), D, 0, 0, 0, xbuf(l + 1), D, p.out1,
                                      p.ldo1, p.y_f32, p.gamma, p.beta, eps, p.mean, p.rstd, d.M, st));
            } else {
                p.kpart = (float*)(ws + W.kpart);
                MFVIT_TRY(gemm_nt_row(d.dtype, REPI_RES_LN, p, st));
            }
        }
    }
    return MFVIT_OK;
}

static int encoder_backward(const mfvit_vit_cfg* cfg, const mfvit_vit_drop* dropcfg, const float* params, const void* shadow, void* workspace,
                            const float* dfeatures, float* dparams, float* dinput, float* dimg, int stage_hi, int stage_lo, mfvit_stream_t stream,
                            bool want_tokens, const mfvit_vit_rel_req* rel = nullptr) {
    Dims d;
    if (!get_dims(cfg, dropcfg, d) || !params || !shadow || !workspace || (!dparams && !dimg && !rel)) return MFVIT_EINVAL;
    if (!d.save || d.tok != want_tokens) return MFVIT_EINVAL;
    if (stage_hi > d.depth || stage_lo < -1 || stage_lo > stage_hi) return MFVIT_EINVAL;
    if (dimg && (d.tok || stage_lo != -1)) return MFVIT_EINVAL;
    const bool wg = dparams != nullptr;
    hipStream_t st = (hipStream_t)stream;
    const ParamLayout L = param_layout(d);
    const ShadowLayout S = shadow_layout(d);
    const WsLayout W = ws_layout(d);
    char* ws = (char*)workspace;
    const char* sh = (const char*)shadow;
    const long D = d.D, F = d.F;
    const long e = d.ep;
    auto xbuf = [&](int l) { return (float*)(ws + W.x0 + (size_t)l * W.x_stride); };
    auto stat = [&](int l) { return (float*)(ws + W.st0 + (size_t)l * W.st_stride); };
    auto blk = [&](int l) { return ws + W.blk0 + (size_t)l * W.blk_stride; };
    auto pblk = [&](int l) { return params + L.blk0 + (long)l * L.blk_stride; };
    auto gblk = [&](int l) { return wg ? dparams + L.blk0 + (long)l * L.blk_stride : nullptr; };
    auto sblk = [&](int l) { return sh + S.blk0 + (size_t)l * S.blk_stride; };
    float* gx = (float*)(ws + W.gx);
    float* gmid = (float*)(ws + W.gmid);
    float* colscr = (float*)(ws + W.colscratch);
    int colpart_used = 0;
    auto next_colpart = [&]() { return (float*)(ws + W.colpart + (size_t)(colpart_used++ % (3 * d.depth + 2)) * W.colpart_stride); };
    ColpartBatch cbatch;
    struct BatchScope {
        ColpartBatch* prev; bool on;
        BatchScope(ColpartBatch* b, bool on_) : on(on_) { if (on) prev = colpart_batch_begin(b); }
        ~BatchScope() { if (on) colpart_batch_begin(prev); }
    } batch_scope(&cbatch, !d.rdrop);
    int tn_used = 0;
    auto next_tnpart = [&]() -> float* {
        return tn_used < TN_SLOTS ? (float*)(ws + W.tnpart + (size_t)(tn_used++) * W.tnpart_stride) : nullptr;
    };
    TnPartBatch tbatch;
    struct TnScope {
        TnPartBatch* prev;
        TnScope(TnPartBatch* b) : prev(tnpart_batch_begin(b)) {}
        ~TnScope() { tnpart_batch_begin(prev); }
    } tn_scope(&tbatch);
    auto pp = [&](size_t off, int l) { return (void*)(ws + off + (size_t)(l & 1) * W.pp_stride); };
    hipStreamCaptureStatus cap = hipStreamCaptureStatusNone;
    const bool capturing = hipStreamIsCapturing(st, &cap) == hipSuccess && cap != hipStreamCaptureStatusNone;
    const bool side_wanted = wg && d.M >= 1024 && d.M <= 4096 && g_wgrad_stream.load(std::memory_order_relaxed) != 0 && !d.rdrop &&
                             !capturing;
    static SideStream no_side;
    SideStream& ss = side_wanted ? side_stream(st) : no_side;
    const bool use_side = side_wanted && ss.ok && W.pp_stride != 0;
    hipStream_t wst = use_side ? ss.s : st;
    auto fork = [&]() -> int {
        if (!use_side) return MFVIT_OK;
        if (hipEventRecord(ss.in, st) != hipSuccess || hipStreamWaitEvent(ss.s, ss.in, 0) != hipSuccess) return MFVIT_ELAUNCH;
        return MFVIT_OK;
    };
    auto wait_layer = [&](int l) -> int {
        if (!use_side || l < 0 || l >= d.depth || l > stage_hi) return MFVIT_OK;
        return hipStreamWaitEvent(st, ss.done[l & 63], 0) == hipSuccess ? MFVIT_OK : MFVIT_ELAUNCH;
    };

    const bool lean_grad = d.dtype == MFVIT_BF16X3 && !d.unfused;
    auto site = [](int l, int which) { return 16u * (unsigned)l + (unsigned)which; };
    const bool rdrop = d.rdrop;
    const DropP off = make_drop(0.f, 0, 0);
    auto dpath = [&](int l, int which) { return make_drop(d.dpr ? d.dpr[l] : 0.f, d.seed, site(l, which)); };
    static int s_domax = INT_MIN;
    const int qdt_bwd = attn_qkv_dtype(d.dtype, d.T, d.HD);
    const bool do_max = env_switch("MFVIT_DO_MAX", 1, s_domax) != 0 && qdt_bwd == MFVIT_X3F16 && (d.HD == 32 || d.HD == 64) && d.T >= 64 && d.D % 128 == 0 && !(d.p_attn > 0.f);
    auto domax = [&](int l) { return (unsigned*)(ws + W.domax) + (size_t)l * d.B * d.H; };
    if (do_max) {
        const int l0 = stage_lo > 0 ? stage_lo : 0, l1 = stage_hi < d.depth - 1 ? stage_hi : d.depth - 1;
        if (l1 >= l0 && hipMemsetAsync(domax(l0), 0, (size_t)(l1 - l0 + 1) * d.B * d.H * 4, st) != hipSuccess) return MFVIT_ELAUNCH;
    }
    for (int s = stage_hi; s >= stage_lo; --s) {
        if (s == d.depth) {
            if (!dfeatures) return MFVIT_EINVAL;
            if (wg)
                MFVIT_TRY(ln_bwd_rows(d.dtype, d.D, dfeatures, D, xbuf(d.depth), D, stat(d.depth), stat(d.depth) + d.M, params + L.norm_w,
                                      nullptr, 0, gx, D, pp(W.gxT, d.depth - 1), D * e, dparams + L.norm_w, dparams + L.norm_b,
                                      rdrop ? colscr + D : gblk(d.depth - 1) + L.fc2_b, next_colpart(), d.M, 1, 0, st));
            else
                MFVIT_TRY(ln_bwd_rows(d.dtype, d.D, dfeatures, D, xbuf(d.depth), D, stat(d.depth), stat(d.depth) + d.M, params + L.norm_w,
                                      nullptr, 0, gx, D, pp(W.gxT, d.depth - 1), D * e, nullptr, nullptr, nullptr, nullptr, d.M, 1, 0, st));
        } else if (s >= 0) {
            const int l = s;
            char* b = blk(l);
            const float* pb = pblk(l);
            float* gb = gblk(l);
            const char* sb = sblk(l);
            void* gxT = pp(W.gxT, l);
            void* gmidT = pp(W.gmidT, l);
            void* dhpre = pp(W.dhpre, l);
            void* dqkv = pp(W.dqkv, l);
            MFVIT_TRY(wait_layer(l + 2));
            GemmP def_tn[2];
            int ndef = 0;
            auto tn_now_or_later = [&](const GemmP& g) -> int {
                if (use_side) { def_tn[ndef++] = g; return MFVIT_OK; }
                return gemm_tn(d.dtype, g, wst);
            };
            const void* gy2 = gxT;
            if (rdrop) {
                MFVIT_TRY(mask_scale_rows(d.dtype, false, gxT, D * e, ws + W.dtmp, D * e, make_drop(d.p_resid, d.seed, site(l, 4)), dpath(l, 7), d.T,
                                          d.M, d.D, st));
                gy2 = ws + W.dtmp;
            }
            if (wg) {
                GemmP p = zero_gemm();
                p.A = gy2; p.lda = D * e; p.W = b + W.hact; p.ldw = F * e;
                p.M = d.M; p.N = d.D; p.K = d.F;
                if (rdrop) p.cs0 = gb + L.fc2_b;
                p.out0 = gb + L.fc2_w; p.ldo0 = F;
                p.cpart = next_tnpart();
                MFVIT_TRY(tn_now_or_later(p));
            }
            {
                GemmP p = zero_gemm();
                p.A = gy2; p.lda = D * e; p.W = sb + S.fc2_t; p.ldw = D * e;
                p.M = d.M; p.N = d.F; p.K = d.D;
                p.aux = b + W.hpre; p.ldaux = F;
                p.out0 = dhpre; p.ldo0 = F * e;
                if (fc1b_in_tile() && wg) { p.cs0 = gb + L.fc1_b; p.cpart = next_colpart(); }
                MFVIT_TRY(gemm_nt_tile(d.dtype, EPI_GELU_BWD, p, st));
            }
            if (wg) {
                GemmP p = zero_gemm();
                p.A = dhpre; p.lda = F * e; p.W = b + W.y2; p.ldw = D * e;
                p.M = d.M; p.N = d.F; p.K = d.D;
                if (!fc1b_in_tile()) p.cs0 = gb + L.fc1_b;
                p.out0 = gb + L.fc1_w; p.ldo0 = D;
                p.cpart = next_tnpart();
                MFVIT_TRY(tn_now_or_later(p));
            }
            {
                GemmP p = zero_gemm();
                p.A = dhpre; p.lda = F * e; p.W = sb + S.fc1_t; p.ldw = F * e;
                p.M = d.M; p.N = d.D; p.K = d.F;
                p.aux = b + W.xmid; p.ldaux = D;
                p.mean = (float*)(b + W.st2); p.rstd = (float*)(b + W.st2) + d.M;
                p.gamma = pb + L.ln2_w;
                if (lean_grad) { p.res_t = gxT; p.ldres_t = D * e; p.out0 = nullptr; }
                else { p.res = gx; p.ldres = D; p.out0 = gmid; }
                p.ldo0 = D; p.out1 = gmidT; p.ldo1 = D * e;
                if (wg) { p.cs0 = gb + L.ln2_w; p.cs1 = gb + L.ln2_b; p.cs2 = rdrop ? colscr + D : gb + L.proj_b; p.cpart = next_colpart(); }
                if (d.unfused) {
                    GemmP q = zero_gemm();
                    q.A = p.A; q.lda = p.lda; q.W = p.W; q.ldw = p.ldw; q.M = p.M; q.N = p.N; q.K = p.K;
                    q.out0 = ws + W.utmp; q.ldo0 = D * e;
                    MFVIT_TRY(gemm_nt_tile(d.dtype, EPI_NONE, q, st));
                    MFVIT_TRY(ln_bwd_rows(d.dtype, d.D, nullptr, 0, (const float*)(b + W.xmid), D, p.mean, p.rstd, p.gamma, gx, D, gmid, D, gmidT, D * e,
                                          p.cs0, p.cs1, p.cs2, p.cpart, d.M, 1, 0, st, ws + W.utmp, D * e));
                } else {
                    p.kpart = (float*)(ws + W.kpart);
                    MFVIT_TRY(gemm_nt_row(d.dtype, REPI_LNBWD_RES, p, st));
                }
            }
            const void* gyp = gmidT;
            if (rdrop) {
                MFVIT_TRY(mask_scale_rows(d.dtype, false, gmidT, D * e, ws + W.dtmp, D * e, make_drop(d.p_resid, d.seed, site(l, 3)), dpath(l, 6), d.T,
                                          d.M, d.D, st));
                gyp = ws + W.dtmp;
            }
            GemmP pend_proj = zero_gemm();
            bool have_pend = false;
            if (wg) {
                GemmP p = zero_gemm();
                p.A = gyp; p.lda = D * e; p.W = b + W.attn; p.ldw = D * e;
                p.M = d.M; p.N = d.D; p.K = d.D;
                if (rdrop) p.cs0 = gb + L.proj_b;
                p.out0 = gb + L.proj_w; p.ldo0 = D;
                p.cpart = next_tnpart();
                if (!rdrop) {
                    pend_proj = p;
                    have_pend = true;
                } else {
                    MFVIT_TRY(gemm_tn(d.dtype, p, wst));
                }
            }
            {
                GemmP p = zero_gemm();
                p.A = gyp; p.lda = D * e; p.W = sb + S.proj_t; p.ldw = D * e;
                p.M = d.M; p.N = d.D; p.K = d.D;
                p.out0 = ws + W.dattn; p.ldo0 = D * e;
                if (do_max) { p.omax = domax(l); p.omax_rows = d.T; p.omax_hd = d.HD; }
                MFVIT_TRY(gemm_nt_tile(d.dtype, EPI_NONE, p, st));
            }
            if (rel && l == 0) {
                MFVIT_TRY(rel_block_step(d, rel, l, qdt_bwd, b + W.qkv, (const float*)(b + W.lse), ws + W.dattn, st));
                continue;
            }
            if (d.p_attn > 0.f)
                MFVIT_TRY(attn_bwd_tiled_drop(d.dtype, b + W.qkv, b + W.attn, ws + W.dattn, (const float*)(b + W.lse), dqkv, d.B, d.T, d.H, d.HD,
                                              make_drop(d.p_attn, d.seed, site(l, 2)), st));
            else
            MFVIT_TRY(attn_bwd(qdt_bwd, b + W.qkv, b + W.attn, ws + W.dattn, (const float*)(b + W.lse), dqkv, nullptr,
                               d.B, d.T, d.H, d.HD, st, do_max ? domax(l) : nullptr));
            if (rel) MFVIT_TRY(rel_block_step(d, rel, l, qdt_bwd, b + W.qkv, (const float*)(b + W.lse), ws + W.dattn, st));
            MFVIT_TRY(fork());
            for (int i = 0; i < ndef; ++i) MFVIT_TRY(gemm_tn(d.dtype, def_tn[i], wst));
            if (wg) {
                GemmP p = zero_gemm();
                p.A = dqkv; p.lda = 3 * D * e; p.W = b + W.y1; p.ldw = D * e;
                p.M = d.M; p.N = 3 * d.D; p.K = d.D;
                p.cs0 = gb + L.qkv_b;
                p.out0 = gb + L.qkv_w; p.ldo0 = D;
                p.cpart = next_tnpart();
                GemmP pend_nc = pend_proj;
                pend_nc.cpart = nullptr;
                if (have_pend && gemm_tn_pair_supported(d.dtype, p, pend_nc)) {
                    MFVIT_TRY(gemm_tn_glds_pair(d.dtype, p, pend_nc, wst));
                } else {
                    if (have_pend) MFVIT_TRY(gemm_tn(d.dtype, pend_proj, wst));
                    MFVIT_TRY(gemm_tn(d.dtype, p, wst));
                }
            }
            MFVIT_TRY(tnpart_batch_flush(wst));
            tn_used = 0;
            if (use_side && hipEventRecord(ss.done[l & 63], ss.s) != hipSuccess) return MFVIT_ELAUNCH;
            MFVIT_TRY(wait_layer(l + 1));
            {
                if (wg && l == 0 && hipMemsetAsync(colscr, 0, 2 * D * sizeof(float), st) != hipSuccess) return MFVIT_ELAUNCH;
                GemmP p = zero_gemm();
                p.A = dqkv; p.lda = 3 * D * e; p.W = sb + S.qkv_t; p.ldw = 3 * D * e;
                p.M = d.M; p.N = d.D; p.K = 3 * d.D;
                p.aux = xbuf(l); p.ldaux = D;
                p.mean = stat(l); p.rstd = stat(l) + d.M;
                p.gamma = pb + L.ln1_w;
                if (lean_grad) { p.res_t = gmidT; p.ldres_t = D * e; p.out0 = l == 0 ? gx : nullptr; }
                else { p.res = gmid; p.ldres = D; p.out0 = gx; }
                p.ldo0 = D; p.out1 = pp(W.gxT, l - 1); p.ldo1 = D * e;
                if (wg) { p.cs0 = gb + L.ln1_w; p.cs1 = gb + L.ln1_b; p.cs2 = (l > 0 && !rdrop) ? gblk(l - 1) + L.fc2_b : colscr; p.cpart = next_colpart(); }
                if (d.unfused) {
                    GemmP q = zero_gemm();
                    q.A = p.A; q.lda = p.lda; q.W = p.W; q.ldw = p.ldw; q.M = p.M; q.N = p.N; q.K = p.K;
                    q.out0 = ws + W.utmp; q.ldo0 = D * e;
                    MFVIT_TRY(gemm_nt_tile(d.dtype, EPI_NONE, q, st));
                    MFVIT_TRY(ln_bwd_rows(d.dtype, d.D, nullptr, 0, xbuf(l), D, p.mean, p.rstd, p.gamma, gmid, D, gx, D, pp(W.gxT, l - 1), D * e,
                                          p.cs0, p.cs1, p.cs2, p.cpart, d.M, 1, 0, st, ws + W.utmp, D * e));
                } else {
                    p.kpart = (float*)(ws + W.kpart);
                    MFVIT_TRY(gemm_nt_row(d.dtype, REPI_LNBWD_RES, p, st));
                }
            }
        } else if (d.tok) {
            MFVIT_TRY(colpart_batch_flush(st));
            if (d.p_embd > 0.f)
                MFVIT_TRY(mask_scale_rows(d.dtype, true, gx, D, gx, D, make_drop(d.p_embd, d.seed, 1), off, 1, d.M, d.D, st));
            if (dinput && hipMemcpyAsync(dinput, gx, (size_t)d.M * D * sizeof(float), hipMemcpyDeviceToDevice, st) != hipSuccess)
                return MFVIT_ELAUNCH;
            if (d.use_pos) MFVIT_TRY(batch_sum(gx, dparams + L.pos, d.B, (long)d.T * D, st));
        } else {
            MFVIT_TRY(colpart_batch_flush(st));
            if (d.p_embd > 0.f) {
                MFVIT_TRY(mask_scale_rows(d.dtype, true, gx, D, gx, D, make_drop(d.p_embd, d.seed, 1), off, 1, d.M, d.D, st));
                MFVIT_TRY(cast_transpose(d.dtype, gx, pp(W.gxT, -1), nullptr, d.M, d.D, st));
                if (wg) {
                    if (hipMemsetAsync(colscr, 0, D * sizeof(float), st) != hipSuccess) return MFVIT_ELAUNCH;
                    MFVIT_TRY(colsum_rows(gx, D, colscr, d.M, 1, 0, d.D, st));
                }
            }
            if (dimg) {
                char* wpeT = ws + W.wpeT;
                MFVIT_TRY(cast_transpose(d.dtype, params + L.pe_w, nullptr, wpeT, d.D, 768, st));
                GemmP p = zero_gemm();
                p.A = (const char*)pp(W.gxT, -1) + (size_t)D * d.es; p.lda = D * e;
                p.W = wpeT; p.ldw = D * e;
                p.M = d.M - 1; p.N = 768; p.K = d.D;
                p.orow_in = d.np; p.orow_out = d.T;
                p.out0 = dimg; p.ldo0 = cfg->img_w;
                MFVIT_TRY(gemm_nt_tile(d.dtype, EPI_COL2IM16, p, st));
            }
            if (!wg) continue;
            MFVIT_TRY(colsum_rows(gx, D, dparams + L.cls, d.B, d.T, 0, d.D, st));
            if (!cfg->stop_grad_conv1) {
                MFVIT_TRY(colsum_rows(gx, D, colscr + D, d.B, d.T, 0, d.D, st));
                MFVIT_TRY(axpy(dparams + L.pe_b, colscr, 1.0f, d.D, st));
                MFVIT_TRY(axpy(dparams + L.pe_b, colscr + D, -1.0f, d.D, st));
                GemmP p = zero_gemm();
                p.A = pp(W.gxT, -1); p.lda = D * e; p.W = ws + W.patches; p.ldw = 768 * e;
                p.M = d.Mp; p.N = d.D; p.K = 768;
                p.orow_in = d.np; p.orow_out = d.T; p.orow_off = 1;
                p.out0 = dparams + L.pe_w; p.ldo0 = 768;
                p.cpart = next_tnpart();
                MFVIT_TRY(fork());
                MFVIT_TRY(gemm_tn(d.dtype, p, wst));
            }
        }
    }
    MFVIT_TRY(colpart_batch_flush(st));
    MFVIT_TRY(tnpart_batch_flush(wst));
    if (use_side) {
        if (hipEventRecord(ss.end, ss.s) != hipSuccess || hipStreamWaitEvent(st, ss.end, 0) != hipSuccess) return MFVIT_ELAUNCH;
    }
    return MFVIT_OK;
}

extern "C" {

int mfvit_vit_forward(const mfvit_vit_cfg* cfg, const float* params, const void* shadow, const float* img, void* workspace,
                      float* features, mfvit_stream_t stream) {
    ShareScope share(cfg);
    return encoder_forward(cfg, nullptr, params, shadow, img, workspace, features, stream, false);
}
int mfvit_vit_forward_drop(const mfvit_vit_cfg* cfg, const mfvit_vit_drop* drop, const float* params, const void* shadow, const float* img,
                           void* workspace, float* features, mfvit_stream_t stream) {
    if (!drop) return MFVIT_EINVAL;
    ShareScope share(cfg);
    return encoder_forward(cfg, drop, params, shadow, img, workspace, features, stream, false);
}
size_t mfvit_vit_attn_scratch_bytes(const mfvit_vit_cfg* cfg, const mfvit_vit_attn_req* req) {
    Dims d;
    if (!attn_req_ok(cfg, req, d)) return 0;
    return req->rollout ? align256((size_t)d.depth * d.B * d.T * (d.T + 1) * 4) : 256;
}
int mfvit_vit_forward_attn(const mfvit_vit_cfg* cfg, const mfvit_vit_attn_req* req, const float* params, const void* shadow, const float* img,
                           void* workspace, float* features, mfvit_stream_t stream) {
    Dims d;
    if (!attn_req_ok(cfg, req, d) || !req->scratch) return MFVIT_EINVAL;
    ShareScope share(cfg);
    MFVIT_TRY(encoder_forward(cfg, nullptr, params, shadow, img, workspace, features, stream, false, req));
    if (req->rollout) MFVIT_TRY(attn_rollout((const float*)req->scratch, attn_scratch_sums(d, req), d.depth, d.B, d.T, req->rollout, (hipStream_t)stream));
    return MFVIT_OK;
}
size_t mfvit_vit_rel_scratch_bytes(const mfvit_vit_cfg* cfg, const mfvit_vit_rel_req* req) {
    Dims d;
    if (!rel_req_ok(cfg, req, d)) return 0;
    return req->relevance ? align256((size_t)d.B * d.T * ((d.T + 31) / 32 + 1) * 4) : 256;
}
int mfvit_vit_backward_rel(const mfvit_vit_cfg* cfg, const mfvit_vit_rel_req* req, const float* params, const void* shadow, void* workspace,
                           const float* dfeatures, mfvit_stream_t stream) {
    Dims d;
    if (!rel_req_ok(cfg, req, d) || !req->scratch || !dfeatures || !params || !shadow || !workspace) return MFVIT_EINVAL;
    ShareScope share(cfg);
    return encoder_backward(cfg, nullptr, params, shadow, workspace, dfeatures, nullptr, nullptr, nullptr, d.depth, 0, stream, false, req);
}
int mfvit_vit_backward(const mfvit_vit_cfg* cfg, const float* params, const void* shadow, void* workspace, const float* dfeatures,
                       float* dparams, int stage_hi, int stage_lo, mfvit_stream_t stream) {
    if (!dparams) return MFVIT_EINVAL;
    ShareScope share(cfg);
    return encoder_backward(cfg, nullptr, params, shadow, workspace, dfeatures, dparams, nullptr, nullptr, stage_hi, stage_lo, stream, false);
}
int mfvit_vit_backward_ex(const mfvit_vit_cfg* cfg, const mfvit_vit_drop* drop, const float* params, const void* shadow, void* workspace,
                          const float* dfeatures, float* dparams, float* dimg, int stage_hi, int stage_lo, mfvit_stream_t stream) {
    ShareScope share(cfg);
    return encoder_backward(cfg, drop, params, shadow, workspace, dfeatures, dparams, nullptr, dimg, stage_hi, stage_lo, stream, false);
}
int mfvit_vit_backward_drop(const mfvit_vit_cfg* cfg, const mfvit_vit_drop* drop, const float* params, const void* shadow, void* workspace,
                            const float* dfeatures, float* dparams, int stage_hi, int stage_lo, mfvit_stream_t stream) {
    if (!drop || !dparams) return MFVIT_EINVAL;
    ShareScope share(cfg);
    return encoder_backward(cfg, drop, params, shadow, workspace, dfeatures, dparams, nullptr, nullptr, stage_hi, stage_lo, stream, false);
}
int mfvit_gpt_forward(const mfvit_vit_cfg* cfg, const float* params, const void* shadow, const float* tokens, void* workspace, float* out,
                      mfvit_stream_t stream) {
    ShareScope share(cfg);
    return encoder_forward(cfg, nullptr, params, shadow, tokens, workspace, out, stream, true);
}
int mfvit_gpt_backward(const mfvit_vit_cfg* cfg, const float* params, const void* shadow, void* workspace, const float* dout, float* dparams,
                       float* dtokens, mfvit_stream_t stream) {
    if (!cfg || !dtokens || !dout) return MFVIT_EINVAL;
    ShareScope share(cfg);
    if (!dparams) return MFVIT_EINVAL;
    return encoder_backward(cfg, nullptr, params, shadow, workspace, dout, dparams, dtokens, nullptr, cfg->depth, -1, stream, true);
}

int mfvit_input_transform(const uint8_t* src, const int64_t* desc, const int32_t* tables, int n, int S, int crop, const float* mean3,
                          const float* std3, float* out, mfvit_stream_t stream) {
    if (!src || !desc || !tables || !mean3 || !std3 || !out) return MFVIT_EINVAL;
    if (crop > S) return MFVIT_EINVAL;
    return input_transform(src, (const long long*)desc, tables, n, S, crop, crop, mean3, std3, out, (hipStream_t)stream);
}
int mfvit_input_transform_rect(const uint8_t* src, const int64_t* desc, const int32_t* tables, int n, int S, int out_h, int out_w,
                               const float* mean3, const float* std3, float* out, mfvit_stream_t stream) {
    if (!src || !desc || !tables || !mean3 || !std3 || !out) return MFVIT_EINVAL;
    return input_transform(src, (const long long*)desc, tables, n, S, out_h, out_w, mean3, std3, out, (hipStream_t)stream);
}
size_t mfvit_input_photometric_workspace_bytes(int n, int S) { return input_photometric_workspace_bytes(n, S); }
int mfvit_input_photometric(const uint8_t* src, const int64_t* desc, const int32_t* tables, const int32_t* photo, int n, int S, int max_radius,
                            void* workspace, const float* mean3, const float* std3, float* out, mfvit_stream_t stream) {
    if (!src || !desc || !tables || !photo || !workspace || !mean3 || !std3 || !out) return MFVIT_EINVAL;
    return input_photometric(src, (const long long*)desc, tables, photo, n, S, max_radius, workspace, mean3, std3, out, (hipStream_t)stream);
}
int mfvit_eval_counts(const float* scores, int64_t ld, const int64_t* labels, int n, int C, uint64_t* confusion, int64_t* preds,
                      uint64_t* u2, uint64_t* npos, mfvit_stream_t stream) {
    if (!scores || !labels || (!confusion && !(u2 && npos))) return MFVIT_EINVAL;
    return eval_counts(scores, ld, labels, n, C, (unsigned long long*)confusion, (unsigned long long*)u2, (unsigned long long*)npos, preds,
                       (hipStream_t)stream);
}
int mfvit_linear_fwd(int dtype, int epilogue, const void* x, int64_t ldx, const void* w, int64_t ldw, const float* bias, void* y,
                     int64_t ldy, void* y2, int64_t ldy2, int M, int N, int K, mfvit_stream_t stream) {
    if (!x || !w || (!y && epilogue != EPI_BIAS_GELU)) return MFVIT_EINVAL;
    if (epilogue != EPI_BIAS && epilogue != EPI_BIAS_GELU && epilogue != EPI_NONE && epilogue != EPI_BIAS_X3F16) return MFVIT_EINVAL;
    if (epilogue == EPI_BIAS_GELU && !y2) return MFVIT_EINVAL;
    GemmP p = zero_gemm();
    p.A = x; p.lda = ldx; p.W = w; p.ldw = ldw; p.M = M; p.N = N; p.K = K;
    p.bias = bias; p.out0 = y; p.ldo0 = ldy; p.out1 = y2; p.ldo1 = ldy2;
    return gemm_nt_tile(dtype, epilogue, p, (hipStream_t)stream);
}
int mfvit_linear_dgrad_act(int dtype, const void* dy, int64_t lddy, const void* wt, int64_t ldwt, const void* act_grad, int64_t ldg,
                           void* dx, int64_t lddx, int M, int N, int K, mfvit_stream_t stream) {
    if (!dy || !wt || !act_grad || !dx) return MFVIT_EINVAL;
    GemmP p = zero_gemm();
    p.A = dy; p.lda = lddy; p.W = wt; p.ldw = ldwt; p.M = M; p.N = N; p.K = K;
    p.aux = act_grad; p.ldaux = ldg; p.out0 = dx; p.ldo0 = lddx;
    return gemm_nt_tile(dtype, EPI_GELU_BWD, p, (hipStream_t)stream);
}
int mfvit_linear_wgrad(int dtype, const void* dy, int64_t lddy, const void* x, int64_t ldx, float* dw, int64_t lddw, int M, int N, int K,
                       mfvit_stream_t stream) {
    if (!dy || !x || !dw) return MFVIT_EINVAL;
    GemmP p = zero_gemm();
    p.A = dy; p.lda = lddy; p.W = x; p.ldw = ldx; p.M = M; p.N = N; p.K = K;
    p.out0 = dw; p.ldo0 = lddw;
    return gemm_tn(dtype, p, (hipStream_t)stream);
}
int mfvit_linear_wgrad_ws(int dtype, const void* dy, int64_t lddy, const void* x, int64_t ldx, float* dw, int64_t lddw, int M, int N,
                          int K, float* scratch, mfvit_stream_t stream) {
    if (!dy || !x || !dw) return MFVIT_EINVAL;
    GemmP p = zero_gemm();
    p.A = dy; p.lda = lddy; p.W = x; p.ldw = ldx; p.M = M; p.N = N; p.K = K;
    p.out0 = dw; p.ldo0 = lddw;
    p.cpart = scratch;
    return gemm_tn(dtype, p, (hipStream_t)stream);
}
int mfvit_linear_wgrad_pair(int dtype, const void* dy_a, int64_t lddy_a, const void* x_a, int64_t ldx_a, float* dw_a, int64_t lddw_a, float* dbias_a,
                            int Na, const void* dy_b, int64_t lddy_b, const void* x_b, int64_t ldx_b, float* dw_b, int64_t lddw_b, int Nb, int M, int K,
                            mfvit_stream_t stream) {
    if (!dy_a || !x_a || !dw_a || !dy_b || !x_b || !dw_b) return MFVIT_EINVAL;
    GemmP a = zero_gemm(), b = zero_gemm();
    a.A = dy_a; a.lda = lddy_a; a.W = x_a; a.ldw = ldx_a; a.M = M; a.N = Na; a.K = K; a.out0 = dw_a; a.ldo0 = lddw_a; a.cs0 = dbias_a;
    b.A = dy_b; b.lda = lddy_b; b.W = x_b; b.ldw = ldx_b; b.M = M; b.N = Nb; b.K = K; b.out0 = dw_b; b.ldo0 = lddw_b;
    if (!gemm_tn_pair_supported(dtype, a, b)) return MFVIT_ENOSYS;
    return gemm_tn_glds_pair(dtype, a, b, (hipStream_t)stream);
}
int mfvit_linear_res_ln_fwd(int dtype, const void* a, int64_t lda, const void* w, int64_t ldw, const float* bias, const float* res,
                            int64_t ldres, float* x_out, void* y, int y_f32, const float* gamma, const float* beta, float eps,
                            float* mean, float* rstd, int M, int K, mfvit_stream_t stream) {
    return mfvit_linear_res_ln_fwd_ws(dtype, a, lda, w, ldw, bias, res, ldres, x_out, y, y_f32, gamma, beta, eps, mean, rstd, M, K, nullptr, stream);
}
int mfvit_linear_res_ln_fwd_ws(int dtype, const void* a, int64_t lda, const void* w, int64_t ldw, const float* bias, const float* res,
                               int64_t ldres, float* x_out, void* y, int y_f32, const float* gamma, const float* beta, float eps,
                               float* mean, float* rstd, int M, int K, float* scratch, mfvit_stream_t stream) {
    if (!a || !w || !y || !gamma || !beta || ((size_t)scratch & 15)) return MFVIT_EINVAL;
    GemmP p = zero_gemm();
    p.kpart = scratch;
    p.A = a; p.lda = lda; p.W = w; p.ldw = ldw; p.M = M; p.N = 384; p.K = K;
    p.bias = bias; p.res = res; p.ldres = ldres;
    p.out0 = x_out; p.ldo0 = 384; p.out1 = y; p.ldo1 = (dtype == MFVIT_BF16X3 && !y_f32) ? 768 : 384; p.y_f32 = y_f32;
    p.gamma = gamma; p.beta = beta; p.eps = eps; p.mean = mean; p.rstd = rstd;
    return gemm_nt_row(dtype, REPI_RES_LN, p, (hipStream_t)stream);
}
int mfvit_linear_dgrad_ln_bwd(int dtype, const void* dy, int64_t lddy, const void* wt, int64_t ldwt, const float* x, const float* mean,
                              const float* rstd, const float* gamma, const float* dres, float* dx, void* dx_t, float* dgamma,
                              float* dbeta, float* dcol, int M, int K, mfvit_stream_t stream) {
    return mfvit_linear_dgrad_ln_bwd_ws(dtype, dy, lddy, wt, ldwt, x, mean, rstd, gamma, dres, dx, dx_t, dgamma, dbeta, dcol, M, K, nullptr, stream);
}
int mfvit_linear_dgrad_ln_bwd_ws(int dtype, const void* dy, int64_t lddy, const void* wt, int64_t ldwt, const float* x, const float* mean,
                                 const float* rstd, const float* gamma, const float* dres, float* dx, void* dx_t, float* dgamma,
                                 float* dbeta, float* dcol, int M, int K, float* scratch, mfvit_stream_t stream) {
    if (!dy || !wt || !x || !mean || !rstd || !gamma || !dx || ((size_t)scratch & 15)) return MFVIT_EINVAL;
    GemmP p = zero_gemm();
    p.kpart = scratch;
    p.A = dy; p.lda = lddy; p.W = wt; p.ldw = ldwt; p.M = M; p.N = 384; p.K = K;
    p.aux = x; p.ldaux = 384; p.mean = (float*)mean; p.rstd = (float*)rstd; p.gamma = gamma;
    p.res = dres; p.ldres = 384;
    p.out0 = dx; p.ldo0 = 384; p.out1 = dx_t; p.ldo1 = dtype == MFVIT_BF16X3 ? 768 : 384;
    p.cs0 = dgamma; p.cs1 = dbeta; p.cs2 = dcol;
    return gemm_nt_row(dtype, REPI_LNBWD_RES, p, (hipStream_t)stream);
}
int mfvit_attention_fwd(int dtype, const void* qkv, void* out, float* lse, int B, int T, int H, int head_dim, mfvit_stream_t stream) {
    if (!qkv || !out || !lse || B <= 0 || T <= 0 || H <= 0) return MFVIT_EINVAL;
    return attn_fwd(dtype, qkv, out, lse, B, T, H, head_dim, (hipStream_t)stream);
}
int mfvit_attention_qkv_dtype(int dtype, int T, int head_dim) { return attn_qkv_dtype(dtype, T, head_dim); }
int mfvit_attention_bwd(int dtype, const void* qkv, const void* out, const void* dout, const float* lse, void* dqkv, float* dbias_qkv,
                        int B, int T, int H, int head_dim, mfvit_stream_t stream) {
    if (!qkv || !out || !dout || !lse || !dqkv || B <= 0 || T <= 0 || H <= 0) return MFVIT_EINVAL;
    return attn_bwd(dtype, qkv, out, dout, lse, dqkv, dbias_qkv, B, T, H, head_dim, (hipStream_t)stream);
}
int mfvit_attention_drop_fwd(int dtype, const void* qkv, void* out, float* lse, int B, int T, int H, int head_dim, float p, uint64_t seed,
                             uint32_t site, mfvit_stream_t stream) {
    if (!qkv || !out || !lse || B <= 0 || T <= 0 || H <= 0 || !(p >= 0.f && p < 1.f)) return MFVIT_EINVAL;
    if (!attn_tiled_supported(dtype, T, head_dim)) return MFVIT_ENOSYS;
    return attn_fwd_tiled_drop(dtype, qkv, out, lse, B, T, H, head_dim, make_drop(p, seed, site), (hipStream_t)stream);
}
int mfvit_attention_drop_bwd(int dtype, const void* qkv, const void* out, const void* dout, const float* lse, void* dqkv, int B, int T, int H,
                             int head_dim, float p, uint64_t seed, uint32_t site, mfvit_stream_t stream) {
    if (!qkv || !out || !dout || !lse || !dqkv || B <= 0 || T <= 0 || H <= 0 || !(p >= 0.f && p < 1.f)) return MFVIT_EINVAL;
    if (!attn_tiled_supported(dtype, T, head_dim)) return MFVIT_ENOSYS;
    return attn_bwd_tiled_drop(dtype, qkv, out, dout, lse, dqkv, B, T, H, head_dim, make_drop(p, seed, site), (hipStream_t)stream);
}
int mfvit_dropout_mask(float p, uint64_t seed, uint32_t site, int64_t n, uint8_t* keep, mfvit_stream_t stream) {
    if (!keep || !(p >= 0.f && p < 1.f)) return MFVIT_EINVAL;
    return dropout_mask(make_drop(p, seed, site), n, keep, (hipStream_t)stream);
}
int mfvit_layernorm_fwd(int dtype, const float* x, void* y, int y_f32, const float* gamma, const float* beta, float eps, float* mean,
                        float* rstd, int rows, int N, mfvit_stream_t stream) {
    if (!x || !y || !gamma || !beta) return MFVIT_EINVAL;
    return ln_rows(dtype, N, x, N, nullptr, 0, 0, nullptr, 0, y, (dtype == MFVIT_BF16X3 && !y_f32) ? 2 * N : N, y_f32, gamma, beta, eps, mean, rstd, rows, 1, 0,
// ... 31 lines not shown
```

### multi-feature-vit_amd/mfvit/_lib.py

```python
import ctypes
import os

import torch
from ctypes import POINTER, Structure, c_char_p, c_double, c_float, c_int, c_int64, c_size_t, c_uint32, c_uint64, c_void_p

_HERE = os.path.dirname(os.path.abspath(__file__))
LIB_PATH = os.environ.get("MFVIT_LIB") or os.path.join(_HERE, "libmfvit_hip.so")
ABI_VERSION = 5

F32, BF16, BF16X3, F16, X3F16 = 0, 1, 2, 3, 4
EPI_BIAS, EPI_BIAS_GELU, EPI_NONE, EPI_BIAS_X3F16 = 0, 1, 3, 5


class VitCfg(Structure):
    _fields_ = [("dtype", c_int), ("batch", c_int), ("img_h", c_int), ("img_w", c_int), ("dim", c_int), ("depth", c_int),
                ("heads", c_int), ("mlp_dim", c_int), ("save_for_backward", c_int), ("stop_grad_conv1", c_int),
                ("ln_eps", c_float), ("token_input", c_int), ("tokens", c_int), ("use_pos", c_int), ("act", c_int),
                ("p_embd", c_float), ("p_attn", c_float), ("p_resid", c_float), ("seed_lo", c_uint32), ("seed_hi", c_uint32),
                ("stream_share", c_int)]


class VitDrop(Structure):
    _fields_ = [("drop", c_float), ("attn_drop", c_float), ("drop_path", POINTER(c_float)), ("seed", c_uint64)]


class VitAttnReq(Structure):
    _fields_ = [("blocks", c_uint64), ("fuse", c_int), ("cls_only", c_int), ("maps", c_void_p), ("rollout", c_void_p), ("scratch", c_void_p)]


HEAD_FUSION = {None: 0, "mean": 1, "max": 2, "min": 3}


class VitRelReq(Structure):
    _fields_ = [("blocks", c_uint64), ("maps", c_void_p), ("relevance", c_void_p), ("scratch", c_void_p)]


class FusionCfg(Structure):
    _fields_ = [("batch", c_int), ("tokens", c_int), ("dim", c_int), ("heads", c_int), ("num_classes", c_int),
                ("eps_pre", c_float), ("eps_post", c_float)]


P = c_void_p
I = c_int
L = c_int64
F = c_float
D = c_double

SIGNATURES = {
    "mfvit_abi_version": (I, []),
    "mfvit_build_info": (c_char_p, []),
    "mfvit_vit_param_count": (c_size_t, [POINTER(VitCfg)]),
    "mfvit_vit_param_layout": (I, [POINTER(VitCfg), POINTER(c_int64)]),
    "mfvit_vit_shadow_bytes": (c_size_t, [POINTER(VitCfg)]),
    "mfvit_vit_prepare_shadow": (I, [POINTER(VitCfg), P, P, P]),
    "mfvit_vit_workspace_bytes": (c_size_t, [POINTER(VitCfg)]),
    "mfvit_vit_forward": (I, [POINTER(VitCfg), P, P, P, P, P, P]),
    "mfvit_vit_backward": (I, [POINTER(VitCfg), P, P, P, P, P, I, I, P]),
    "mfvit_vit_workspace_bytes_drop": (c_size_t, [POINTER(VitCfg), POINTER(VitDrop)]),
    "mfvit_vit_forward_drop": (I, [POINTER(VitCfg), POINTER(VitDrop), P, P, P, P, P, P]),
    "mfvit_vit_backward_drop": (I, [POINTER(VitCfg), POINTER(VitDrop), P, P, P, P, P, I, I, P]),
    "mfvit_vit_workspace_bytes_ex": (c_size_t, [POINTER(VitCfg), POINTER(VitDrop), I]),
    "mfvit_vit_backward_ex": (I, [POINTER(VitCfg), POINTER(VitDrop), P, P, P, P, P, P, I, I, P]),
    "mfvit_vit_attn_scratch_bytes": (c_size_t, [POINTER(VitCfg), POINTER(VitAttnReq)]),
    "mfvit_vit_forward_attn": (I, [POINTER(VitCfg), POINTER(VitAttnReq), P, P, P, P, P, P]),
    "mfvit_vit_rel_scratch_bytes": (c_size_t, [POINTER(VitCfg), POINTER(VitRelReq)]),
    "mfvit_vit_backward_rel": (I, [POINTER(VitCfg), POINTER(VitRelReq), P, P, P, P, P]),
    "mfvit_gpt_forward": (I, [POINTER(VitCfg), P, P, P, P, P, P]),
    "mfvit_gpt_backward": (I, [POINTER(VitCfg), P, P, P, P, P, P, P]),
    "mfvit_linear_fwd": (I, [I, I, P, L, P, L, P, P, L, P, L, I, I, I, P]),
    "mfvit_linear_dgrad_act": (I, [I, P, L, P, L, P, L, P, L, I, I, I, P]),
    "mfvit_linear_wgrad": (I, [I, P, L, P, L, P, L, I, I, I, P]),
    "mfvit_linear_wgrad_ws": (I, [I, P, L, P, L, P, L, I, I, I, P, P]),
    "mfvit_linear_wgrad_pair": (I, [I, P, L, P, L, P, L, P, I, P, L, P, L, P, L, I, I, I, P]),
    "mfvit_linear_res_ln_fwd": (I, [I, P, L, P, L, P, P, L, P, P, I, P, P, F, P, P, I, I, P]),
    "mfvit_linear_dgrad_ln_bwd": (I, [I, P, L, P, L, P, P, P, P, P, P, P, P, P, P, I, I, P]),
    "mfvit_linear_res_ln_fwd_ws": (I, [I, P, L, P, L, P, P, L, P, P, I, P, P, F, P, P, I, I, P, P]),
    "mfvit_linear_dgrad_ln_bwd_ws": (I, [I, P, L, P, L, P, P, P, P, P, P, P, P, P, P, I, I, P, P]),
    "mfvit_attention_fwd": (I, [I, P, P, P, I, I, I, I, P]),
    "mfvit_attention_bwd": (I, [I, P, P, P, P, P, P, I, I, I, I, P]),
    "mfvit_attention_qkv_dtype": (I, [I, I, I]),
    "mfvit_attention_drop_fwd": (I, [I, P, P, P, I, I, I, I, F, c_uint64, c_uint32, P]),
    "mfvit_attention_drop_bwd": (I, [I, P, P, P, P, P, I, I, I, I, F, c_uint64, c_uint32, P]),
    "mfvit_dropout_mask": (I, [F, c_uint64, c_uint32, L, P, P]),
    "mfvit_layernorm_fwd": (I, [I, P, P, I, P, P, F, P, P, I, I, P]),
    "mfvit_layernorm_bwd": (I, [I, P, P, P, P, P, P, P, P, P, P, P, I, I, P]),
    "mfvit_cast_transpose": (I, [I, P, P, P, I, I, P]),
    "mfvit_head_fwd": (I, [P, L, P, P, P, L, I, I, I, I, P]),
    "mfvit_head_bwd": (I, [P, L, P, L, P, P, L, I, P, P, I, I, I, P]),
    "mfvit_cross_entropy": (I, [P, P, P, P, P, I, I, P]),
    "mfvit_cross_entropy_soft": (I, [P, P, P, P, F, P, P, P, I, I, P]),
    "mfvit_batch_mix": (I, [P, P, P, P, P, P, I, I, I, I, P]),
    "mfvit_fusion_param_count": (c_size_t, [POINTER(FusionCfg)]),
    "mfvit_fusion_workspace_bytes": (c_size_t, [POINTER(FusionCfg)]),
    "mfvit_fusion_forward": (I, [POINTER(FusionCfg), P, P, P, P, P, P, P, P, P, P, P, P]),
    "mfvit_fusion_ex_param_count": (c_size_t, [POINTER(FusionCfg), I, I]),
    "mfvit_fusion_ex_workspace_bytes": (c_size_t, [POINTER(FusionCfg), I, I]),
    "mfvit_fusion_ex_forward": (I, [POINTER(FusionCfg), I, I, P, P, P, P, P, P, P, P, P, P, P, P]),
    "mfvit_fusion_ex_backward": (I, [POINTER(FusionCfg), I, I, P, P, P, P, P, P, P, P, P, P, P, P, P, P, P, P, P]),
    "mfvit_bn_stats": (I, [I, P, I, I, P, P, P]),
    "mfvit_bn_combine": (I, [P, P, P, I, I, F, F, P, P, P, P, P]),
    "mfvit_bn_apply": (I, [I, P, P, P, P, P, I, P, I, I, P]),
    "mfvit_bn_bwd_sums": (I, [I, P, P, P, P, P, I, I, I, P, P, P]),
    "mfvit_bn_bwd_apply": (I, [I, P, P, P, P, P, P, I, P, P, F, P, I, I, P]),
    "mfvit_l2norm_fwd": (I, [P, P, P, I, I, F, P]),
    "mfvit_l2norm_bwd": (I, [P, P, P, P, I, I, P]),
    "mfvit_rowdot": (I, [P, P, P, L, F, I, I, P]),
    "mfvit_cross_entropy_rows": (I, [P, L, P, P, P, P, L, I, I, P]),
    "mfvit_ema_update": (I, [P, P, F, L, P]),
    "mfvit_lars_step": (I, [P, I, I, P, F, F, F, F, P]),
    "mfvit_adam_step": (I, [P, I, F, F, F, F, F, I, P]),
    "mfvit_sgd_step": (I, [P, I, F, F, F, I, P]),
    "mfvit_amp_unscale": (I, [P, I, F, P, P]),
    "mfvit_grad_norm_partials": (I, [P, I, I, P, P]),
    "mfvit_grad_clip_coef": (I, [P, P, I, I, I, D, P, P, P]),
    "mfvit_grad_scale": (I, [P, I, P, P]),
    "mfvit_prenorm_xattn_forward": (I, [POINTER(FusionCfg), P, P, P, P, P, P]),
    "mfvit_prenorm_xattn_backward": (I, [POINTER(FusionCfg), P, P, P, P, P, P, P, P, P]),
    "mfvit_xattn_forward": (I, [POINTER(FusionCfg), P, P, P, P, P]),
    "mfvit_xattn_backward": (I, [POINTER(FusionCfg), P, P, P, P, P, P, P]),
    "mfvit_input_transform": (I, [P, P, P, I, I, I, P, P, P, P]),
    "mfvit_input_transform_rect": (I, [P, P, P, I, I, I, I, P, P, P, P]),
    "mfvit_input_photometric_workspace_bytes": (c_size_t, [I, I]),
    "mfvit_input_photometric": (I, [P, P, P, P, I, I, I, P, P, P, P, P]),
    "mfvit_eval_counts": (I, [P, L, P, I, I, P, P, P, P, P]),
    "mfvit_prof_enable": (I, [I]),
    "mfvit_set_wgrad_stream": (I, [I]),
    "mfvit_set_stream_share": (I, [I]),
    "mfvit_prof_collect": (I, [POINTER(ctypes.c_double), I]),
    "mfvit_prof_collect_tags": (I, [POINTER(ctypes.c_double), I]),
    "mfvit_prof_class_name": (c_char_p, [I]),
    "mfvit_fusion_backward": (I, [POINTER(FusionCfg), P, P, P, P, P, P, P, P, P, P, P, P, P, P, P, P, P]),
}

_lib = None


class MfvitError(RuntimeError):
    pass


def lib():
    global _lib
    if _lib is not None:
        return _lib
    if not os.path.exists(LIB_PATH):
        raise MfvitError(
            f"libmfvit_hip.so not found at {LIB_PATH}. Build it with `python -c 'import __graft_entry__ as g; g.build()'` "
            "(hipcc --offload-arch=gfx950). There is no CPU/eager fallback for the MF-ViT hot path.")
    try:
        h = ctypes.CDLL(LIB_PATH)
    except OSError as e:
        raise MfvitError(f"cannot load {LIB_PATH}: {e}") from e
    abi = h.mfvit_abi_version()
    if abi != ABI_VERSION:
        raise MfvitError(f"{LIB_PATH} has C ABI {abi}, this package expects ABI {ABI_VERSION}: rebuild the library")
    for name, (res, args) in SIGNATURES.items():
        fn = getattr(h, name)
        fn.restype = res
        fn.argtypes = args
    _lib = h
    return h


def source_hash():
    import hashlib
    h = hashlib.sha1()
    csrc = os.path.join(os.path.dirname(_HERE), "csrc")
    files = sorted(os.path.join(csrc, f) for f in os.listdir(csrc) if f.endswith((".hip", ".cuh", ".h")))
    files.append(os.path.join(os.path.dirname(os.path.dirname(_HERE)), "include", "mfvit.h"))
    for f in files:
        h.update(os.path.basename(f).encode())
        with open(f, "rb") as fh:
            h.update(fh.read())
    return h.hexdigest()


def check(rc, what):
    if rc != 0:
        raise MfvitError(f"{what} failed with code {rc} (-22 = invalid argument, -5 = launch error, -38 = not built for this dtype / size)")


def ptr(t):
    return None if t is None else t.data_ptr()


def stream():
    import torch
    return torch.cuda.current_stream().cuda_stream


def require_cuda(*tensors):
    for t in tensors:
        if t is not None and not t.is_cuda:
            raise MfvitError("MF-ViT HIP ops need tensors on a ROCm GPU ('cuda' device); there is no CPU fallback")


PRECISIONS = ("bf16x3", "bf16", "fp16", "fp32")


def dtype_code(precision):
    if precision in ("bf16x3", "split", "split-bf16"):
        return BF16X3
    if precision in ("bf16", "bfloat16"):
        return BF16
    if precision in ("fp16", "f16", "float16", "half"):
        return F16
    if precision in ("fp32", "f32", "float32"):
        return F32
    raise ValueError(f"precision must be one of {PRECISIONS}, got {precision!r}")
```

### multi-feature-vit_amd/mfvit/encoder.py

```python
import contextlib
import ctypes
import math
import operator
import os

import torch
import torch.nn as nn

from . import _lib, ops
from ._lib import VitCfg, check, lib, ptr, stream


def default_precision():
    return os.environ.get("MFVIT_PRECISION", "bf16x3")


def build_2d_sincos_position_embedding(gh, gw, dim, temperature=10000.0):
    assert dim % 4 == 0, "embed dim must be divisible by 4 for the 2-D sin-cos position embedding"
    gw_, gh_ = torch.meshgrid(torch.arange(gw, dtype=torch.float64), torch.arange(gh, dtype=torch.float64), indexing="ij")
    pos_dim = dim // 4
    omega = 1.0 / (temperature ** (torch.arange(pos_dim, dtype=torch.float64) / pos_dim))
    out_w = gw_.flatten()[:, None] * omega[None]
    out_h = gh_.flatten()[:, None] * omega[None]
    pe = torch.cat([out_w.sin(), out_w.cos(), out_h.sin(), out_h.cos()], dim=1)[None]
# ... 267 lines not shown

    def _arena_intact(self):
        base = self._arena.data_ptr()
        f32 = torch.float32
        for (_, mod, attr), off in zip(self._param_holders(), self._arena_offsets):
            p = mod._parameters[attr]
            if p.data_ptr() != base + 4 * off or p.dtype != f32:
                return False
        return True

    def _apply(self, fn, *a, **k):
        out = super()._apply(fn, *a, **k)
        self._flatten()
        return out

    def flat_parameters(self):
        if not self._arena_intact():
            self._flatten()
        return self._arena

    def arena_slice(self, name):
        return self._offsets[name]

    def block_slice(self, i):
        a = self._offsets[f"blocks.{i}.norm1.weight"][0]
        o, n = self._offsets[f"blocks.{i}.mlp.fc2.bias"]
        return a, o + n - a

    def drop_rates(self):
        blocks = list(self._modules["blocks"]._modules.values())
        drop = float(self._modules["pos_drop"].p)
        attn = float(blocks[0]._modules["attn"]._modules["attn_drop"].p)
        dpr = []
        for b in blocks:
            a, mlp = b._modules["attn"]._modules, b._modules["mlp"]._modules
            if float(a["proj_drop"].p) != drop or float(mlp["drop"].p) != drop or float(a["attn_drop"].p) != attn:
                raise _lib.MfvitError("the encoder kernels take one drop_rate (pos_drop, proj_drop, mlp.drop) and one attn_drop_rate for all "
                                      "blocks: set the rate-carrier modules consistently")
            dpr.append(float(getattr(b._modules["drop_path"], "drop_prob", 0.0)))
        for r in [drop, attn] + dpr:
            if not 0.0 <= r < 1.0:
                raise _lib.MfvitError(f"dropout rates must lie in [0, 1), got {r}")
        return drop, attn, dpr

    def is_stochastic(self):
        if not self.training:
            return False
        drop, attn, dpr = self.drop_rates()
        return drop > 0.0 or attn > 0.0 or any(r > 0.0 for r in dpr)

    def _draw_drop(self):
        if not self.training:
            return None
        drop, attn, dpr = self.drop_rates()
        if not (drop > 0.0 or attn > 0.0 or any(r > 0.0 for r in dpr)):
            return None
        if _lib.dtype_code(self.precision) == _lib.F32:
            raise _lib.MfvitError("dropout / drop path inside the encoder is built for precision 'bf16x3' (f32-grade), 'bf16' and 'fp16', not 'fp32': "
                                  "use one of those, or train with the rates at 0")
        seed = int(torch.randint(0, 2 ** 62, (1,), dtype=torch.int64).item())
        rates = (ctypes.c_float * len(dpr))(*dpr)
        d = _lib.VitDrop(drop, attn, ctypes.cast(rates, ctypes.POINTER(ctypes.c_float)), seed)
        d._rates = rates
        self._last_drop = d
        return d

    def _cfg(self, img, save):
        c = VitCfg()
        c.dtype = _lib.dtype_code(self.precision)
        c.batch, _, c.img_h, c.img_w = img.shape
        c.dim, c.depth, c.heads, c.mlp_dim = self.embed_dim, self.depth, self.num_heads, self.mlp_dim
        c.save_for_backward = int(bool(save))
        c.stop_grad_conv1 = int(not self.patch_embed.proj.weight.requires_grad)
        c.ln_eps = 1e-6
        c.stream_share = int(getattr(self, "_stream_share", 0))
        return c

    def _param_version(self):
        return sum(p._version for p in self._arena_params)

    def _ensure_shadow(self, cfg):
        key = (self._param_version(), cfg.dtype, str(self._arena.device))
        if self._shadow is not None and key == self._shadow_key:
            return
        if not self._arena_intact():
            self._flatten()
            key = (self._param_version(), cfg.dtype, str(self._arena.device))
        nbytes = lib().mfvit_vit_shadow_bytes(cfg)
        if self._shadow is None or self._shadow.numel() != nbytes:
            self._shadow = torch.empty(nbytes, device=self._arena.device, dtype=torch.uint8)
        check(lib().mfvit_vit_prepare_shadow(cfg, ptr(self._arena), ptr(self._shadow), stream()), "mfvit_vit_prepare_shadow")
        self._shadow_key = key
        self._feat_cache = None

    def _get_ws(self, cfg, drop=None, want_dimg=False):
        if want_dimg:
            nbytes = lib().mfvit_vit_workspace_bytes_ex(cfg, drop, 1)
        else:
            nbytes = lib().mfvit_vit_workspace_bytes(cfg) if drop is None else lib().mfvit_vit_workspace_bytes_drop(cfg, drop)
        if nbytes == 0:
            raise _lib.MfvitError("invalid encoder configuration (image size must be a multiple of 16, dim 384 or 768, head_dim 32 / 64 / 96)")
        pool = self._ws_pool.setdefault(nbytes, [])
        return pool.pop() if pool else torch.empty(nbytes, device=self._arena.device, dtype=torch.uint8)

    def _release_ws(self, ws):
        if ws is not None:
            pool = self._ws_pool.setdefault(ws.numel(), [])
            if len(pool) < 2:
                pool.append(ws)

    def _prep_img(self, img):
        _lib.require_cuda(img)
        if img.dtype != torch.float32:
            img = img.float()
        img = img.contiguous()
        if img.shape[1] != 3 or (img.shape[2], img.shape[3]) != self.img_size:
            raise _lib.MfvitError(f"expected (B,3,{self.img_size[0]},{self.img_size[1]}) images, got {tuple(img.shape)} "
                                  "(pos_embed is size-bound)")
        if self._arena.device != img.device:
            raise _lib.MfvitError(f"model on {self._arena.device} but input on {img.device}")
        return img

    def _run_forward(self, img, save, drop=None, want_dimg=False):
        img = self._prep_img(img)
        cfg = self._cfg(img, save)
        self._ensure_shadow(cfg)
        ws = self._get_ws(cfg, drop, want_dimg)
        feats = torch.empty(img.shape[0], self.num_tokens, self.embed_dim, device=img.device, dtype=torch.float32)
        if drop is None:
            check(lib().mfvit_vit_forward(cfg, ptr(self._arena), ptr(self._shadow), ptr(img), ptr(ws), ptr(feats), stream()),
                  "mfvit_vit_forward")
        else:
            check(lib().mfvit_vit_forward_drop(cfg, drop, ptr(self._arena), ptr(self._shadow), ptr(img), ptr(ws), ptr(feats), stream()),
                  "mfvit_vit_forward_drop")
        if not save:
            self._release_ws(ws)
            ws = None
        return feats, ws

    def _run_backward(self, cfg, ws, dfeats, on_stage_done=None, drop=None, dimg=None, want_params=True):
        dfeats = dfeats.contiguous()
        if dfeats.dtype != torch.float32:
            dfeats = dfeats.float()
        if not want_params:
            if dimg is None:
                raise _lib.MfvitError("a backward without parameter gradients needs the image gradient")
            check(lib().mfvit_vit_backward_ex(cfg, drop, ptr(self._arena), ptr(self._shadow), ptr(ws), ptr(dfeats), None, ptr(dimg),
                                              self.depth, -1, stream()), "mfvit_vit_backward_ex")
            return [None] * len(self._arena_params)
        reuse = getattr(self, "reuse_grad_arena", os.environ.get("MFVIT_GRAD_ARENA_REUSE", "1") != "0")
        ga = getattr(self, "_grad_arena", None) if reuse else None
        if (ga is not None and not getattr(self, "_grad_arena_lent", False) and ga.shape == self._arena.shape
                and ga.device == self._arena.device and all(p.grad is None for p in self._arena_params)):
            gflat = ga.zero_()
        else:
            gflat = torch.zeros_like(self._arena)
            if not getattr(self, "_grad_arena_lent", False):
                self._grad_arena = gflat
        self._grad_arena_lent = True
        hook = on_stage_done or getattr(self, "_grad_stage_hook", None)

        def bwd(hi, lo):
            if dimg is not None and lo == -1:
                check(lib().mfvit_vit_backward_ex(cfg, drop, ptr(self._arena), ptr(self._shadow), ptr(ws), ptr(dfeats), ptr(gflat), ptr(dimg),
                                                  hi, lo, stream()), "mfvit_vit_backward_ex")
            elif drop is None:
                check(lib().mfvit_vit_backward(cfg, ptr(self._arena), ptr(self._shadow), ptr(ws), ptr(dfeats), ptr(gflat), hi, lo, stream()),
                      "mfvit_vit_backward")
            else:
                check(lib().mfvit_vit_backward_drop(cfg, drop, ptr(self._arena), ptr(self._shadow), ptr(ws), ptr(dfeats), ptr(gflat), hi, lo,
                                                    stream()), "mfvit_vit_backward_drop")
        if hook is None:
            bwd(self.depth, -1)
        else:
            gb = max(1, int(getattr(self, "_grad_bucket_layers", 4)))
            hi = self.depth
            while hi >= -1:
                lo = max(hi - gb, -1) if hi == self.depth else max(hi - gb + 1, -1)
                if lo == 0:
                    lo = -1
                bwd(hi, lo)
                hook(self, hi, lo, gflat)
                hi = lo - 1
        self._last_grad_arena = gflat
        params = [mod._parameters[attr] for _, mod, attr in self._param_holders()]
        views = torch._utils._unflatten_dense_tensors(gflat, params)
        return [v if p.requires_grad else None for v, p in zip(views, params)]

    def _features(self, x, caller):
        need_x = torch.is_grad_enabled() and x.requires_grad
        need = need_x or (torch.is_grad_enabled() and any(p.requires_grad for p in self._arena_params))
        key = (x._version, need, need_x, self._param_version(), torch.is_grad_enabled())
        c = self._feat_cache
        self._feat_cache = None
        drop = self._draw_drop()
        stochastic = drop is not None
        if c is not None and c[0] is x and c[1] == key and c[2] != caller and not stochastic:
            return c[3]
        c = None
        self._grad_arena_lent = False
        feats = _EncoderFn.apply(self, x, need, drop, *self._arena_params)
        self._feat_cache = None if stochastic else (x, key, caller, feats)
        return feats

    def features3D(self, x):
        return self._features(x, "features3D")

    def forward_head(self, feats):
        h = self.head
        if isinstance(h, nn.Linear) and h.weight.dtype == torch.float32 and feats.is_cuda:
            return _HeadFn.apply(feats, h.weight, h.bias)
        return h(feats[:, 0])

    def forward(self, x):
        return self.forward_head(self._features(x, "forward"))

    def _attn_blocks(self, blocks):
        if blocks is None:
            return list(range(self.depth))
        out = set()
        for i in blocks:
            try:
                if isinstance(i, bool):
                    raise TypeError
                i = operator.index(i)
            except TypeError:
                raise ValueError(f"block indices must be integers, got {i!r}") from None
            if not -self.depth <= i < self.depth:
                raise ValueError(f"block index {i} out of range for depth {self.depth}")
            out.add(i % self.depth)
        if not out:
            raise ValueError("no block requested")
        return sorted(out)

    def _attn_forward(self, x, blocks, fuse, cls_only, rollout):
        img = self._prep_img(x.detach())
        with torch.no_grad():
            cfg = self._cfg(img, False)
            cache = self._feat_cache
            self._ensure_shadow(cfg)
            self._feat_cache = cache
            B, T, H = img.shape[0], self.num_tokens, self.num_heads
            rows = 1 if cls_only else T
            per = B * (1 if fuse else H) * rows * T
            dev = img.device
            maps = torch.empty(len(blocks) * per, device=dev, dtype=torch.float32) if blocks else None
            roll = torch.empty(B, T - 1, device=dev, dtype=torch.float32) if rollout else None
            req = _lib.VitAttnReq(sum(1 << l for l in blocks), fuse, int(cls_only), ptr(maps), ptr(roll), None)
            nbytes = lib().mfvit_vit_attn_scratch_bytes(cfg, req)
            if nbytes == 0:
                raise _lib.MfvitError("invalid attention-map request for this encoder configuration")
            scratch = torch.empty(nbytes, device=dev, dtype=torch.uint8)
            req.scratch = scratch.data_ptr()
            ws = self._get_ws(cfg)
            feats = torch.empty(B, T, self.embed_dim, device=dev, dtype=torch.float32)
            try:
                check(lib().mfvit_vit_forward_attn(cfg, req, ptr(self._arena), ptr(self._shadow), ptr(img), ptr(ws), ptr(feats), stream()),
                      "mfvit_vit_forward_attn")
            finally:
                self._release_ws(ws)
        shape = ((B,) if fuse else (B, H)) + ((T,) if cls_only else (T, T))
        return [maps[i * per:(i + 1) * per].view(shape) for i in range(len(blocks))], roll

    def get_attention_maps(self, x, blocks=None, head_fusion=None, cls_only=False):
        if head_fusion not in _lib.HEAD_FUSION:
            raise ValueError(f"head_fusion must be None, 'mean', 'max' or 'min', got {head_fusion!r}")
        blocks = self._attn_blocks(blocks)
        return self._attn_forward(x, blocks, _lib.HEAD_FUSION[head_fusion], bool(cls_only), False)[0]

    def get_last_selfattention(self, x):
        return self.get_attention_maps(x, blocks=[self.depth - 1])[0]

    def attention_rollout(self, x, head_fusion="mean"):
        if head_fusion not in ("mean", "max", "min"):
            raise ValueError(f"head_fusion must be 'mean', 'max' or 'min', got {head_fusion!r}")
        _, roll = self._attn_forward(x, [], _lib.HEAD_FUSION[head_fusion], False, True)
        return roll.view(roll.shape[0], self.img_size[0] // 16, self.img_size[1] // 16)

    def _head_width(self):
        h = self.head
        for m in reversed(list(h.modules())):
            for a in ("out_features", "num_features"):
                v = getattr(m, a, None)
                if isinstance(v, int) and not isinstance(v, bool):
                    return v
        return None

    def _rel_forward(self, x):
        img = self._prep_img(x.detach())
        with torch.no_grad():
            cfg = self._cfg(img, True)
            cache = self._feat_cache
            self._ensure_shadow(cfg)
            self._feat_cache = cache
            ws = self._get_ws(cfg)
            feats = torch.empty(img.shape[0], self.num_tokens, self.embed_dim, device=img.device, dtype=torch.float32)
            try:
                check(lib().mfvit_vit_forward(cfg, ptr(self._arena), ptr(self._shadow), ptr(img), ptr(ws), ptr(feats), stream()),
                      "mfvit_vit_forward")
            except BaseException:
                self._release_ws(ws)
                raise
        return cfg, ws, feats

    def _rel_backward(self, cfg, ws, dfeats, blocks, want_rel):
        B, T = cfg.batch, self.num_tokens
        dev = ws.device
        dfeats = dfeats.detach().float().contiguous()
        per = B * T * T
        with torch.no_grad():
            maps = torch.empty(len(blocks) * per, device=dev, dtype=torch.float32) if blocks else None
            rel = torch.empty(B, T - 1, device=dev, dtype=torch.float32) if want_rel else None
            req = _lib.VitRelReq(sum(1 << l for l in blocks), ptr(maps), ptr(rel), None)
            nbytes = lib().mfvit_vit_rel_scratch_bytes(cfg, req)
            if nbytes == 0:
                raise _lib.MfvitError("invalid relevance request for this encoder configuration")
            scratch = torch.empty(nbytes, device=dev, dtype=torch.uint8)
            req.scratch = scratch.data_ptr()
# ... 25 lines not shown
```

Baseline: 5004.

## Overwrite gradient arena in backward reductions instead of zeroing then accumulating

When the reused gradient arena is handed to backward, the Python side no longer zeroes it. Backward instead runs in a store mode where the reduction kernels write their results directly rather than read-modify-add. Outputs that would still be accumulated get a targeted memset first. The cls, position and patch-bias column sums are fused into one colsum kernel with a minuend output, replacing two axpy launches. This removes a full-arena zero fill and some read traffic, but every gradient destination must be written exactly once, and any missed path would leave stale values.

```diff
diff --git a/include/mfvit.h b/include/mfvit.h
--- a/include/mfvit.h
+++ b/include/mfvit.h
@@ -72,6 +72,11 @@
 size_t mfvit_vit_workspace_bytes_ex(const mfvit_vit_cfg* cfg, const mfvit_vit_drop* drop, int want_dimg);
 int mfvit_vit_backward_ex(const mfvit_vit_cfg* cfg, const mfvit_vit_drop* drop, const float* params, const void* shadow, void* workspace,
                           const float* dfeatures, float* dparams, float* dimg, int stage_hi, int stage_lo, mfvit_stream_t stream);
+
+#define MFVIT_BWD_OVERWRITE 1u
+int mfvit_vit_backward_flags(const mfvit_vit_cfg* cfg, const mfvit_vit_drop* drop, const float* params, const void* shadow, void* workspace,
+                             const float* dfeatures, float* dparams, float* dimg, int stage_hi, int stage_lo, unsigned flags,
+                             mfvit_stream_t stream);
 
 typedef struct mfvit_vit_attn_req {
     uint64_t blocks;
diff --git a/multi-feature-vit_amd/csrc/elementwise.hip b/multi-feature-vit_amd/csrc/elementwise.hip
--- a/multi-feature-vit_amd/csrc/elementwise.hip
+++ b/multi-feature-vit_amd/csrc/elementwise.hip
@@ -571,17 +571,9 @@
     MFVIT_CHECK_LAUNCH();
     return MFVIT_OK;
 }
-__global__ void axpy_kernel(float* __restrict__ y, const float* __restrict__ x, float a, long n) {
-    const long i = blockIdx.x * (long)blockDim.x + threadIdx.x;
-    if (i < n) y[i] = fmaf(a, x[i], y[i]);
-}
-int axpy(float* y, const float* x, float a, long n, hipStream_t st) {
-    MFVIT_LAUNCH(axpy_kernel, dim3((unsigned)((n + 255) / 256)), dim3(256), 0, st, y, x, a, n);
-    MFVIT_CHECK_LAUNCH();
-    return MFVIT_OK;
-}
 __global__ __launch_bounds__(1024) void colsum_rows_kernel(const float* __restrict__ x, long ld, float* __restrict__ out, int rows,
-                                                           int row_stride, int row_off, int N) {
+                                                           int row_stride, int row_off, int N, int store, const float* __restrict__ minuend,
+                                                           float* __restrict__ out2) {
     const int n = blockIdx.x * 64 + (threadIdx.x & 63), sub = threadIdx.x >> 6;
     __shared__ float sm[16][64];
     float s = 0.f;
@@ -595,24 +587,26 @@
         s = 0.f;
 #pragma unroll
         for (int i = 0; i < 16; ++i) s += sm[i][threadIdx.x];
-        out[n] += s;
-    }
-}
-int colsum_rows(const float* x, long ld, float* out, int rows, int row_stride, int row_off, int N, hipStream_t st) {
-    MFVIT_LAUNCH(colsum_rows_kernel, dim3((N + 63) / 64), dim3(1024), 0, st, x, ld, out, rows, row_stride, row_off, N);
-    MFVIT_CHECK_LAUNCH();
-    return MFVIT_OK;
-}
-
-__global__ __launch_bounds__(256) void batch_sum_kernel(const float* __restrict__ x, float* __restrict__ out, int B, long n) {
+        out[n] = (store ? 0.f : out[n]) + s;
+        if (out2) out2[n] = ((store ? 0.f : out2[n]) + minuend[n]) - s;
+    }
+}
+int colsum_rows(const float* x, long ld, float* out, int rows, int row_stride, int row_off, int N, hipStream_t st, const float* minuend, float* out2) {
+    if ((minuend == nullptr) != (out2 == nullptr)) return MFVIT_EINVAL;
+    MFVIT_LAUNCH(colsum_rows_kernel, dim3((N + 63) / 64), dim3(1024), 0, st, x, ld, out, rows, row_stride, row_off, N, (int)reduce_store_mode(), minuend, out2);
+    MFVIT_CHECK_LAUNCH();
+    return MFVIT_OK;
+}
+
+__global__ __launch_bounds__(256) void batch_sum_kernel(const float* __restrict__ x, float* __restrict__ out, int B, long n, int store) {
     const long i = blockIdx.x * 256L + threadIdx.x;
     if (i >= n) return;
     float s = 0.f;
     for (int b = 0; b < B; ++b) s += x[(long)b * n + i];
-    out[i] += s;
+    out[i] = (store ? 0.f : out[i]) + s;
 }
 int batch_sum(const float* x, float* out, int B, long n, hipStream_t st) {
-    MFVIT_LAUNCH(batch_sum_kernel, dim3((unsigned)((n + 255) / 256)), dim3(256), 0, st, x, out, B, n);
+    MFVIT_LAUNCH(batch_sum_kernel, dim3((unsigned)((n + 255) / 256)), dim3(256), 0, st, x, out, B, n, (int)reduce_store_mode());
     MFVIT_CHECK_LAUNCH();
     return MFVIT_OK;
 }
diff --git a/multi-feature-vit_amd/csrc/gemm.hip b/multi-feature-vit_amd/csrc/gemm.hip
--- a/multi-feature-vit_amd/csrc/gemm.hip
+++ b/multi-feature-vit_amd/csrc/gemm.hip
@@ -915,7 +915,7 @@
 }
 
 __global__ __launch_bounds__(256) void tn_reduce_kernel(const float* __restrict__ part, int splits, long stride, int N, int K, float* __restrict__ out,
-                                                        long ldo) {
+                                                        long ldo, int store) {
     const long q = (long)blockIdx.x * 256 + threadIdx.x;
     const long total4 = (long)N * K / 4;
     if (q >= total4) return;
@@ -927,7 +927,7 @@
     }
     const int n = (int)(e / K), k = (int)(e % K);
     float4* o = (float4*)(out + (long)n * ldo + k);
-    float4 c = *o;
+    float4 c = store ? make_float4(0.f, 0.f, 0.f, 0.f) : *o;
     c.x += s.x, c.y += s.y, c.z += s.z, c.w += s.w;
     *o = c;
 }
@@ -948,7 +948,7 @@
     }
     const int n = (int)(e / j.K), k = (int)(e % j.K);
     float4* o = (float4*)(j.out + (long)n * j.ldo + k);
-    float4 c = *o;
+    float4 c = j.store ? make_float4(0.f, 0.f, 0.f, 0.f) : *o;
     c.x += s.x, c.y += s.y, c.z += s.z, c.w += s.w;
     *o = c;
 }
@@ -1051,6 +1051,12 @@
     }
     if (p.nb > 1 || p.splits < 2 || p.ldo0 % 4 || (long)tiles * p.splits > 384) p.cpart = nullptr;
     p.kpart = p.cpart && p.cs0 && (long)tiles * p.splits + 2 <= 384 && p.N % 4 == 0 && (size_t)p.cs0 % 16 == 0 ? p.cpart + (long)p.splits * p.N * p.K : nullptr;
+    if (reduce_store_mode()) {
+        if (p.nb > 1) return MFVIT_EINVAL;
+        int rc = p.cpart ? MFVIT_OK : tn_store_clear((float*)p.out0, p.ldo0, p.N, p.K, st);
+        if (rc == MFVIT_OK && p.cs0 && !p.kpart) rc = tn_store_clear(p.cs0, p.N, 1, p.N, st);
+        if (rc != MFVIT_OK) return rc;
+    }
     ProfScope ps(PROF_GEMM_TN, 2.0 * p.M * p.N * p.K * (p.nb > 1 ? p.nb : 1), 0, st);
     const dim3 grid = xcd1d ? dim3(tiles * p.splits, 1, 1) : dim3(tiles, p.splits, p.nb > 1 ? p.nb : 1);
     if (p.orow_in)
@@ -1066,6 +1072,19 @@
     return MFVIT_OK;
 }
 
+static thread_local bool g_reduce_store = false;
+bool reduce_store_mode(bool on) {
+    const bool prev = g_reduce_store;
+    g_reduce_store = on;
+    return prev;
+}
+bool reduce_store_mode() { return g_reduce_store; }
+int tn_store_clear(float* out, long ldo, int N, int K, hipStream_t st) {
+    if (!out || N <= 0 || K <= 0) return MFVIT_OK;
+    if (ldo != K && N != 1) return MFVIT_EINVAL;
+    return hipMemsetAsync(out, 0, (size_t)N * K * sizeof(float), st) == hipSuccess ? MFVIT_OK : MFVIT_ELAUNCH;
+}
+
 static thread_local TnPartBatch* g_tnpart_batch = nullptr;
 TnPartBatch* tnpart_batch_begin(TnPartBatch* b) {
     TnPartBatch* prev = g_tnpart_batch;
@@ -1089,12 +1108,12 @@
             if (rc != MFVIT_OK) return rc;
         }
         TnPartJob& j = b->job[b->n++];
-        j.part = part; j.out = out; j.stride = stride; j.ldo = ldo; j.splits = splits; j.N = N; j.K = K; j.first4 = b->total4;
+        j.part = part; j.out = out; j.stride = stride; j.ldo = ldo; j.splits = splits; j.N = N; j.K = K; j.store = g_reduce_store; j.first4 = b->total4;
         b->total4 += (long)N * K / 4;
         return MFVIT_OK;
     }
     const long total4 = (long)N * K / 4;
-    MFVIT_LAUNCH(tn_reduce_kernel, dim3((unsigned)((total4 + 255) / 256)), dim3(256), 0, st, part, splits, stride, N, K, out, ldo);
+    MFVIT_LAUNCH(tn_reduce_kernel, dim3((unsigned)((total4 + 255) / 256)), dim3(256), 0, st, part, splits, stride, N, K, out, ldo, (int)g_reduce_store);
     MFVIT_CHECK_LAUNCH();
     return MFVIT_OK;
 }
@@ -1114,14 +1133,15 @@
     return s;
 }
 __global__ __launch_bounds__(64 * CPR_SUB) void colpart_reduce_kernel(const float* __restrict__ part, int G, int ncols, int nq, float* d0, float* d1,
-                                                                     float* d2) {
+                                                                     float* d2, int store) {
     const int c = blockIdx.x * 64 + (threadIdx.x & 63), sub = threadIdx.x >> 6;
     __shared__ float sm[CPR_SUB][64];
     const bool ok = c < nq * ncols;
     float s = colpart_rows(part, ok ? G : 0, (long)nq * ncols, c, sub, sm);
     if (sub == 0 && ok) {
         float* d = c / ncols == 0 ? d0 : (c / ncols == 1 ? d1 : d2);
-        if (d) atomicAdd(d + c % ncols, s);
+        if (d && store) d[c % ncols] = 0.f + s;
+        else if (d) atomicAdd(d + c % ncols, s);
     }
 }
 #define MFVIT_TRY_RC(expr) do { int rc__ = (expr); if (rc__ != MFVIT_OK) return rc__; } while (0)
@@ -1133,7 +1153,8 @@
     float s = colpart_rows(j.part, ok ? j.G : 0, (long)j.nq * j.ncols, c, sub, sm);
     if (sub == 0 && ok) {
         float* d = j.d[c / j.ncols];
-        if (d) atomicAdd(d + c % j.ncols, s);
+        if (d && j.store) d[c % j.ncols] = 0.f + s;
+        else if (d) atomicAdd(d + c % j.ncols, s);
     }
 }
 static thread_local ColpartBatch* g_colpart_batch = nullptr;
@@ -1157,10 +1178,10 @@
     if (ColpartBatch* b = g_colpart_batch) {
         if (b->n == ColpartBatch::MAXJ) MFVIT_TRY_RC(colpart_batch_flush(st));
         ColpartJob& j = b->job[b->n++];
-        j.part = part; j.G = G; j.ncols = ncols; j.nq = nq; j.d[0] = d0; j.d[1] = d1; j.d[2] = d2;
+        j.part = part; j.G = G; j.ncols = ncols; j.nq = nq; j.d[0] = d0; j.d[1] = d1; j.d[2] = d2; j.store = g_reduce_store;
         return MFVIT_OK;
     }
-    MFVIT_LAUNCH(colpart_reduce_kernel, dim3((nq * ncols + 63) / 64), dim3(64 * CPR_SUB), 0, st, part, G, ncols, nq, d0, d1, d2);
+    MFVIT_LAUNCH(colpart_reduce_kernel, dim3((nq * ncols + 63) / 64), dim3(64 * CPR_SUB), 0, st, part, G, ncols, nq, d0, d1, d2, (int)g_reduce_store);
     MFVIT_CHECK_LAUNCH();
     return MFVIT_OK;
 }
diff --git a/multi-feature-vit_amd/csrc/gemm_small.hip b/multi-feature-vit_amd/csrc/gemm_small.hip
--- a/multi-feature-vit_amd/csrc/gemm_small.hip
+++ b/multi-feature-vit_amd/csrc/gemm_small.hip
@@ -162,6 +162,11 @@
 }
 int gemm_tn_small(GemmP p, hipStream_t st) {
     const int nb = p.nb > 1 ? p.nb : 1;
+    if (reduce_store_mode()) {
+        if (nb > 1) return MFVIT_EINVAL;
+        const int rc = tn_store_clear((float*)p.out0, p.ldo0, p.N, p.K, st);
+        if (rc != MFVIT_OK) return rc;
+    }
     ProfScope ps(PROF_OTHER, 2.0 * p.M * p.N * p.K * nb, 0, st);
     MFVIT_LAUNCH(gemm_tn_small_kernel, dim3((p.K + 31) / 32, (p.N + 31) / 32, nb), dim3(256), 0, st, p);
     MFVIT_CHECK_LAUNCH();
diff --git a/multi-feature-vit_amd/csrc/gemm_tn2.hip b/multi-feature-vit_amd/csrc/gemm_tn2.hip
--- a/multi-feature-vit_amd/csrc/gemm_tn2.hip
+++ b/multi-feature-vit_amd/csrc/gemm_tn2.hip
@@ -384,6 +384,12 @@
     }
     if (p.splits < 2 || p.ldo0 % 4 || (p.res_mod && p.ldo1 % 4) || (long)tiles * p.splits > 384) p.cpart = nullptr;
     p.kpart = p.cpart && p.cs0 && (long)tiles * p.splits + 2 <= 384 && p.N % 4 == 0 && (size_t)p.cs0 % 16 == 0 ? p.cpart + (long)p.splits * (p.N + p.res_mod) * p.K : nullptr;
+    if (reduce_store_mode()) {
+        int rc = p.cpart ? MFVIT_OK : tn_store_clear((float*)p.out0, p.ldo0, p.N, p.K, st);
+        if (rc == MFVIT_OK && !p.cpart && p.res_mod) rc = tn_store_clear((float*)p.out1, p.ldo1, p.res_mod, p.K, st);
+        if (rc == MFVIT_OK && p.cs0 && !p.kpart) rc = tn_store_clear(p.cs0, p.N, 1, p.N, st);
+        if (rc != MFVIT_OK) return rc;
+    }
     constexpr int bytes = (is_split<T>::value ? T2_NSP : T2_NS) * T2_STAGE;
     p.rows_per_wg = 0;
     ProfScope ps(PROF_GEMM_TN, 2.0 * p.M * (p.N + p.res_mod) * p.K, 0, st);
diff --git a/multi-feature-vit_amd/csrc/kernels.h b/multi-feature-vit_amd/csrc/kernels.h
--- a/multi-feature-vit_amd/csrc/kernels.h
+++ b/multi-feature-vit_amd/csrc/kernels.h
@@ -33,17 +33,20 @@
 bool gemm_tn_glds_supported(int dtype, const GemmP& p);
 int gemm_tn_glds(int dtype, GemmP p, hipStream_t st);
 int colpart_reduce(const float* part, int G, int ncols, int nq, float* d0, float* d1, float* d2, hipStream_t st);
-struct ColpartJob { const float* part; float* d[3]; int G, ncols, nq; };
+struct ColpartJob { const float* part; float* d[3]; int G, ncols, nq, store; };
 struct ColpartBatch { static constexpr int MAXJ = 48; int n; ColpartJob job[MAXJ]; };
 ColpartBatch* colpart_batch_begin(ColpartBatch* b);
 int colpart_batch_flush(hipStream_t st);
 bool gemm_tn_pair_supported(int dtype, const GemmP& a, const GemmP& b);
 int gemm_tn_glds_pair(int dtype, GemmP a, const GemmP& b, hipStream_t st);
 int tn_partial_reduce(const float* part, int splits, long stride, int N, int K, float* out, long ldo, hipStream_t st);
-struct TnPartJob { const float* part; float* out; long stride, ldo; int splits, N, K; long first4; };
+struct TnPartJob { const float* part; float* out; long stride, ldo; int splits, N, K, store; long first4; };
 struct TnPartBatch { static constexpr int MAXJ = 56; int n; long total4; TnPartJob job[MAXJ]; };
 TnPartBatch* tnpart_batch_begin(TnPartBatch* b);
 int tnpart_batch_flush(hipStream_t st);
+bool reduce_store_mode(bool on);
+bool reduce_store_mode();
+int tn_store_clear(float* out, long ldo, int N, int K, hipStream_t st);
 
 int attn_fwd_exact(int dtype, const void* qkv, void* out, float* lse, int B, int Tn, int H, int HD, hipStream_t st);
 int attn_bwd_exact(int dtype, const void* qkv, const void* out, const void* dout, const float* lse, void* dqkv, float* dbias, int B, int Tn,
@@ -73,8 +76,8 @@
                      float* db, int M, int N, int K, hipStream_t st);
 int ce_small(const float* logits, const long* target, float* loss_mean, float* dlogits, long* preds, int B, int C, hipStream_t st);
 int add_rows(float* dst, long ldd, const float* src, long lds_, int rows, int N, hipStream_t st);
-int axpy(float* y, const float* x, float a, long n, hipStream_t st);
-int colsum_rows(const float* x, long ld, float* out, int rows, int row_stride, int row_off, int N, hipStream_t st);
+int colsum_rows(const float* x, long ld, float* out, int rows, int row_stride, int row_off, int N, hipStream_t st, const float* minuend = nullptr,
+                float* out2 = nullptr);
 int batch_sum(const float* x, float* out, int B, long n, hipStream_t st);
 
 int attn_fwd_tiled_drop(int dtype, const void* qkv, void* out, float* lse, int B, int Tn, int H, int HDim, DropP drop, hipStream_t st);
diff --git a/multi-feature-vit_amd/csrc/vit.hip b/multi-feature-vit_amd/csrc/vit.hip
--- a/multi-feature-vit_amd/csrc/vit.hip
+++ b/multi-feature-vit_amd/csrc/vit.hip
@@ -594,7 +594,7 @@
 
 static int encoder_backward(const mfvit_vit_cfg* cfg, const mfvit_vit_drop* dropcfg, const float* params, const void* shadow, void* workspace,
                             const float* dfeatures, float* dparams, float* dinput, float* dimg, int stage_hi, int stage_lo, mfvit_stream_t stream,
-                            bool want_tokens, const mfvit_vit_rel_req* rel = nullptr) {
+                            bool want_tokens, const mfvit_vit_rel_req* rel = nullptr, bool overwrite = false) {
     Dims d;
     if (!get_dims(cfg, dropcfg, d) || !params || !shadow || !workspace || (!dparams && !dimg && !rel)) return MFVIT_EINVAL;
     if (!d.save || d.tok != want_tokens) return MFVIT_EINVAL;
@@ -618,6 +618,20 @@
     float* gx = (float*)(ws + W.gx);
     float* gmid = (float*)(ws + W.gmid);
     float* colscr = (float*)(ws + W.colscratch);
+    const bool store = overwrite && wg && !d.rdrop;
+    struct StoreScope {
+        bool prev;
+        StoreScope(bool on) : prev(reduce_store_mode(on)) {}
+        ~StoreScope() { reduce_store_mode(prev); }
+    } store_scope(store);
+    if (overwrite && wg && !store) {
+        const int l0 = stage_lo > 0 ? stage_lo : 0, l1 = stage_hi < d.depth - 1 ? stage_hi : d.depth - 1;
+        if (l1 >= l0 && hipMemsetAsync(dparams + L.blk0 + (long)l0 * L.blk_stride, 0, (size_t)(l1 - l0 + 1) * L.blk_stride * sizeof(float), (hipStream_t)stream) != hipSuccess)
+            return MFVIT_ELAUNCH;
+        if (stage_hi == d.depth && hipMemsetAsync(dparams + L.norm_w, 0, (size_t)(L.total - L.norm_w) * sizeof(float), (hipStream_t)stream) != hipSuccess)
+            return MFVIT_ELAUNCH;
+        if (stage_lo == -1 && hipMemsetAsync(dparams, 0, (size_t)L.blk0 * sizeof(float), (hipStream_t)stream) != hipSuccess) return MFVIT_ELAUNCH;
+    }
     int colpart_used = 0;
     auto next_colpart = [&]() { return (float*)(ws + W.colpart + (size_t)(colpart_used++ % (3 * d.depth + 2)) * W.colpart_stride); };
     ColpartBatch cbatch;
@@ -867,11 +881,12 @@
                 MFVIT_TRY(gemm_nt_tile(d.dtype, EPI_COL2IM16, p, st));
             }
             if (!wg) continue;
-            MFVIT_TRY(colsum_rows(gx, D, dparams + L.cls, d.B, d.T, 0, d.D, st));
-            if (!cfg->stop_grad_conv1) {
-                MFVIT_TRY(colsum_rows(gx, D, colscr + D, d.B, d.T, 0, d.D, st));
-                MFVIT_TRY(axpy(dparams + L.pe_b, colscr, 1.0f, d.D, st));
-                MFVIT_TRY(axpy(dparams + L.pe_b, colscr + D, -1.0f, d.D, st));
+            if (store && hipMemsetAsync(dparams + L.pos, 0, (size_t)((cfg->stop_grad_conv1 ? L.blk0 : L.pe_w) - L.pos) * sizeof(float), st) != hipSuccess)
+                return MFVIT_ELAUNCH;
+            if (cfg->stop_grad_conv1) {
+                MFVIT_TRY(colsum_rows(gx, D, dparams + L.cls, d.B, d.T, 0, d.D, st));
+            } else {
+                MFVIT_TRY(colsum_rows(gx, D, dparams + L.cls, d.B, d.T, 0, d.D, st, colscr, dparams + L.pe_b));
                 GemmP p = zero_gemm();
                 p.A = pp(W.gxT, -1); p.lda = D * e; p.W = ws + W.patches; p.ldw = 768 * e;
                 p.M = d.Mp; p.N = d.D; p.K = 768;
@@ -940,6 +955,13 @@
                           const float* dfeatures, float* dparams, float* dimg, int stage_hi, int stage_lo, mfvit_stream_t stream) {
     ShareScope share(cfg);
     return encoder_backward(cfg, drop, params, shadow, workspace, dfeatures, dparams, nullptr, dimg, stage_hi, stage_lo, stream, false);
+}
+int mfvit_vit_backward_flags(const mfvit_vit_cfg* cfg, const mfvit_vit_drop* drop, const float* params, const void* shadow, void* workspace,
+                             const float* dfeatures, float* dparams, float* dimg, int stage_hi, int stage_lo, unsigned flags, mfvit_stream_t stream) {
+    if (flags & ~(unsigned)MFVIT_BWD_OVERWRITE) return MFVIT_EINVAL;
+    ShareScope share(cfg);
+    return encoder_backward(cfg, drop, params, shadow, workspace, dfeatures, dparams, nullptr, dimg, stage_hi, stage_lo, stream, false, nullptr,
+                            (flags & MFVIT_BWD_OVERWRITE) != 0);
 }
 int mfvit_vit_backward_drop(const mfvit_vit_cfg* cfg, const mfvit_vit_drop* drop, const float* params, const void* shadow, void* workspace,
                             const float* dfeatures, float* dparams, int stage_hi, int stage_lo, mfvit_stream_t stream) {
diff --git a/multi-feature-vit_amd/mfvit/_lib.py b/multi-feature-vit_amd/mfvit/_lib.py
--- a/multi-feature-vit_amd/mfvit/_lib.py
+++ b/multi-feature-vit_amd/mfvit/_lib.py
@@ -28,6 +28,7 @@
     _fields_ = [("blocks", c_uint64), ("fuse", c_int), ("cls_only", c_int), ("maps", c_void_p), ("rollout", c_void_p), ("scratch", c_void_p)]
 
 
+BWD_OVERWRITE = 1
 HEAD_FUSION = {None: 0, "mean": 1, "max": 2, "min": 3}
 
 
@@ -61,6 +62,7 @@
     "mfvit_vit_backward_drop": (I, [POINTER(VitCfg), POINTER(VitDrop), P, P, P, P, P, I, I, P]),
     "mfvit_vit_workspace_bytes_ex": (c_size_t, [POINTER(VitCfg), POINTER(VitDrop), I]),
     "mfvit_vit_backward_ex": (I, [POINTER(VitCfg), POINTER(VitDrop), P, P, P, P, P, P, I, I, P]),
+    "mfvit_vit_backward_flags": (I, [POINTER(VitCfg), POINTER(VitDrop), P, P, P, P, P, P, I, I, ctypes.c_uint, P]),
     "mfvit_vit_attn_scratch_bytes": (c_size_t, [POINTER(VitCfg), POINTER(VitAttnReq)]),
     "mfvit_vit_forward_attn": (I, [POINTER(VitCfg), POINTER(VitAttnReq), P, P, P, P, P, P]),
     "mfvit_vit_rel_scratch_bytes": (c_size_t, [POINTER(VitCfg), POINTER(VitRelReq)]),
diff --git a/multi-feature-vit_amd/mfvit/encoder.py b/multi-feature-vit_amd/mfvit/encoder.py
--- a/multi-feature-vit_amd/mfvit/encoder.py
+++ b/multi-feature-vit_amd/mfvit/encoder.py
@@ -443,18 +443,18 @@
         ga = getattr(self, "_grad_arena", None) if reuse else None
         if (ga is not None and not getattr(self, "_grad_arena_lent", False) and ga.shape == self._arena.shape
                 and ga.device == self._arena.device and all(p.grad is None for p in self._arena_params)):
-            gflat = ga.zero_()
+            gflat, flags = ga, _lib.BWD_OVERWRITE
         else:
-            gflat = torch.zeros_like(self._arena)
+            gflat, flags = torch.zeros_like(self._arena), 0
             if not getattr(self, "_grad_arena_lent", False):
                 self._grad_arena = gflat
         self._grad_arena_lent = True
         hook = on_stage_done or getattr(self, "_grad_stage_hook", None)
 
         def bwd(hi, lo):
-            if dimg is not None and lo == -1:
-                check(lib().mfvit_vit_backward_ex(cfg, drop, ptr(self._arena), ptr(self._shadow), ptr(ws), ptr(dfeats), ptr(gflat), ptr(dimg),
-                                                  hi, lo, stream()), "mfvit_vit_backward_ex")
+            if flags or (dimg is not None and lo == -1):
+                check(lib().mfvit_vit_backward_flags(cfg, drop, ptr(self._arena), ptr(self._shadow), ptr(ws), ptr(dfeats), ptr(gflat),
+                                                     ptr(dimg) if lo == -1 else None, hi, lo, flags, stream()), "mfvit_vit_backward_flags")
             elif drop is None:
                 check(lib().mfvit_vit_backward(cfg, ptr(self._arena), ptr(self._shadow), ptr(ws), ptr(dfeats), ptr(gflat), hi, lo, stream()),
                       "mfvit_vit_backward")
```

After: 5023 (median of 6 runs). About the same (+0.4%).
